# JettHuang/jet-pbrt

Hardware: AMD Instinct MI355X
Metric: Msamples/sec (whole node) + per-pixel L2 vs CPU ref, cornell_box 1024spp (higher is better)
Workload: dtype f32

## Files before the change

include/jetpbrt_amd.h:

```cpp
#ifndef JETPBRT_AMD_H
#define JETPBRT_AMD_H
#include <stdint.h>

#ifdef __cplusplus
extern "C" {
#endif

#define JP_ABI_VERSION 7

typedef enum JpStatus {
    JP_OK = 0,
    JP_ERR_INVALID_ARGUMENT = -1,
    JP_ERR_NO_DEVICE = -2,
    JP_ERR_DEVICE = -3,
    JP_ERR_NO_SCENE = -4,
    JP_ERR_UNSUPPORTED = -5
} JpStatus;

enum { JP_SHAPE_TRIANGLE = 0, JP_SHAPE_RECTANGLE = 1, JP_SHAPE_SPHERE = 2, JP_SHAPE_DISK = 3 };
enum { JP_MAT_MATTE = 0, JP_MAT_MIRROR = 1, JP_MAT_GLASS = 2, JP_MAT_PLASTIC = 3, JP_MAT_METAL = 4 };
enum { JP_LIGHT_ENVIRONMENT = 0, JP_LIGHT_AREA = 1, JP_LIGHT_POINT = 2, JP_LIGHT_DIRECTION = 3 };
enum { JP_SAMPLER_STOCK_MT19937 = 0, JP_SAMPLER_COUNTER = 1,
       JP_SAMPLER_DEBUG = 2 };
enum { JP_INTEGRATOR_PATH = 0, JP_INTEGRATOR_WHITTED = 1, JP_INTEGRATOR_DEBUG_NORMAL = 2 };
// ... 296 lines not shown
} JpTexSamplingInfo;
int  jp_set_texture_sampling(JpContext* ctx, const JpTextureSampling* sampling);
int  jp_check_texture_sampling(const JpTextureSampling* sampling, int32_t* n_active_textures, int32_t* n_active_maps);
int  jp_get_texture_sampling_info(JpContext* ctx, JpTexSamplingInfo* out);
int  jp_texture_lookup(const JpTexSampler* s_or_null, int32_t w, int32_t h, const uint8_t* rgb8, int32_t n, const float* uv, uint8_t* rgb8_out);
int  jp_perturb_normals_sampled(const JpTexSampler* s_or_null, int32_t n, const float* nb, const float* ng, const float* dpdu, const float* dpdv, const float* uv,
                                int32_t width, int32_t height, const uint8_t* rgb8, float strength, float* ns_out, int32_t* perturbed_out);

enum { JP_MIP_OFF = 0, JP_MIP_TRILINEAR = 1 };
typedef struct JpTextureMipmaps { int32_t struct_bytes, n_textures; const int32_t* mode; float footprint_scale, bounce_spread; } JpTextureMipmaps;
typedef struct JpTextureMipmapInfo {
    int32_t struct_bytes, n_on;
    int32_t n_levels;
    int32_t mip_last_render;
    int64_t pyramid_bytes_device;
    int64_t cone_bytes_device;
    double  build_ms;
    double  texel_ms;
    float   footprint_scale, bounce_spread, gamma0;
} JpTextureMipmapInfo;
int  jp_set_texture_mipmaps(JpContext* ctx, const JpTextureMipmaps* mipmaps);
int  jp_check_texture_mipmaps(const JpTextureMipmaps* mipmaps, int32_t* n_on);
int  jp_get_texture_mipmap_info(JpContext* ctx, JpTextureMipmapInfo* out);
int  jp_read_mip_chain(JpContext* ctx, int32_t texture, uint8_t* rgb8_out, int64_t capacity);
int  jp_build_mip_chain(int32_t w, int32_t h, const uint8_t* rgb8, uint8_t* rgb8_out, int32_t* level_w, int32_t* level_h, int32_t* n_levels);
int  jp_mip_cone_step(float gamma0, float bounce_spread, int32_t n, const int32_t* flags, const float* t, float* state_inout );
int  jp_mip_footprint(int32_t n, const float* width, const float* area, int32_t w, int32_t h, float scale_u, float scale_v, float footprint_scale, float* rho_out);
int  jp_texture_lookup_mip(const JpTexSampler* s_or_null, int32_t w, int32_t h, const uint8_t* rgb8, int32_t n, const float* uv, const float* rho, uint8_t* rgb8_out);
int  jp_mip_probe(JpContext* ctx, int32_t n, const float* origin, const float* dir, const float* tmin, const float* tmax, const int32_t* flags, float* state_inout,
                  int32_t* prim, float* rho, uint8_t* rgb8);

typedef struct JpLens { int32_t struct_bytes; float radius, focus_distance; int32_t blades; float rotation_deg; } JpLens;
int  jp_set_lens(JpContext* ctx, const JpLens* lens);
typedef struct JpLensInfo { int32_t struct_bytes; float radius, focus_distance; int32_t blades; float rotation_deg; int32_t lens_last_render; } JpLensInfo;
int  jp_get_lens_info(JpContext* ctx, JpLensInfo* out);
int  jp_check_lens(const JpLens* lens);
int  jp_lens_plan(const JpCamera* camera, const JpLens* lens, void* plan_out, int64_t capacity, int64_t* bytes);
int  jp_lens_rays(const JpCamera* camera, const JpLens* lens, int32_t n, const float* fxfy, const float* u, float* origin, float* dir);
int  jp_camera_rays(JpContext* ctx, const JpRenderParams* params, int32_t n, const int32_t* x, const int32_t* y, const int32_t* s, float* origin, float* dir, int32_t* dim_next);
int  jp_focus_distance(JpContext* ctx, float fx, float fy, float* focus_out);

typedef struct JpFilm { int32_t struct_bytes; int32_t hdr; float sample_clamp; } JpFilm;
int  jp_set_film(JpContext* ctx, const JpFilm* film);
int  jp_check_film(const JpFilm* film);
typedef struct JpFilmInfo { int32_t struct_bytes, hdr; float sample_clamp; int32_t hdr_last_render; } JpFilmInfo;
int  jp_get_film_info(JpContext* ctx, JpFilmInfo* out);
int  jp_film_samples(const JpFilm* film, int32_t n, const float* in_rgb, float* out_rgb);

#define JP_FILM_BINS 256
int  jp_film_histogram(JpContext* ctx, int32_t width, int32_t height, const float* film_rgb, uint32_t* hist);
int  jp_film_histogram_device(JpContext* ctx, int32_t width, int32_t height, const void* film_dev, void* hist_dev, int sync);

enum { JP_CURVE_CLAMP = 0, JP_CURVE_REINHARD = 1, JP_CURVE_ACES = 2, JP_CURVE_HABLE = 3 };
enum { JP_EXPOSURE_MANUAL = 0, JP_EXPOSURE_AUTO = 1 };
typedef struct JpToneMap { int32_t struct_bytes, curve, exposure_mode; float ev, key, white, pct_low, pct_high; } JpToneMap;
int  jp_set_tonemap(JpContext* ctx, const JpToneMap* tonemap);
int  jp_check_tonemap(const JpToneMap* tonemap);
int  jp_exposure_from_histogram(const JpToneMap* tonemap, const uint32_t* hist, float* scale_out);
int  jp_tonemap(JpContext* ctx, const JpToneMap* tonemap, int32_t width, int32_t height, const float* film_rgb, uint8_t* rgb8_out, float* rgb_out, float* scale_out);
int  jp_tonemap_device(JpContext* ctx, const JpToneMap* tonemap, int32_t width, int32_t height, const void* film_dev, void* rgb8_dev, void* rgb_dev, float* scale_out, int sync);
int  jp_tonemap_host(const JpToneMap* tonemap, float scale, int64_t n_values, const float* in, uint8_t* rgb8_out, float* rgb_out);
typedef struct JpToneMapInfo { int32_t struct_bytes, curve, exposure_mode; float scale_last; int32_t mapped_last_render; double histogram_ms, tonemap_ms; } JpToneMapInfo;
int  jp_get_tonemap_info(JpContext* ctx, JpToneMapInfo* out);

#define JP_UPLOAD_TABLES 11
typedef struct JpUploadTable { int64_t bytes; uint64_t fnv1a; } JpUploadTable;
typedef struct JpUploadInfo {
    int32_t struct_bytes;
    int32_t trav_mode;
    int32_t stack_depth, stack_depth_q4;
    int64_t lds_bytes, lds_bytes_shadow, shade_lds_bytes;
    int32_t scene_in_lds, tables_in_lds, shade_prims_in_lds, stage_nee, n_planes;
    int32_t persist, vote, shade_sort, use_q4, q4_shadow, cert;
    int32_t class_mask, shape_mask, light_mask, light_shape_mask;
    int32_t has_null_material, stack_lds_words;
    int32_t n_nodes, n_prims, n_flat, n_wide, n_q4;
    int32_t bvh_nodes, bvh_height;
    int32_t wide_height, q4_height, cert_eye_leaves, n_env;
    float   cert_pad, cert_pad_eye, env_sum[3];
    JpUploadTable table[JP_UPLOAD_TABLES];
} JpUploadInfo;
int  jp_describe_upload(const JpOptions* options_or_null, int32_t light_mode, const JpScene* scene, JpUploadInfo* out);

enum { JP_TABLE_NODES = 0, JP_TABLE_PRIMS = 1, JP_TABLE_META = 2, JP_TABLE_WIDE = 7, JP_TABLE_Q4 = 8, JP_TABLE_FLAT = 10 };
typedef struct JpTreeInfo {
    int32_t struct_bytes;
    int32_t n_prims, n_nodes, bvh_height;
    int32_t n_wide, wide_height;
    int32_t n_q4, q4_height;
    int32_t n_flat;
} JpTreeInfo;
int  jp_copy_upload_table(const JpOptions* options_or_null, int32_t light_mode, const JpScene* scene, int32_t which, void* out, int64_t capacity_bytes, int64_t* bytes);
int  jp_read_scene_table(JpContext* ctx, int32_t which, void* out, int64_t capacity_bytes, int64_t* bytes);
int  jp_get_tree_info(JpContext* ctx, JpTreeInfo* out);

#ifdef __cplusplus
}
#endif
#endif
```

jet-pbrt_amd/__init__.py:

```python
import ctypes as C
import os

PKG_DIR = os.path.dirname(os.path.abspath(__file__))
REPO_DIR = os.path.dirname(PKG_DIR)
HIP_LIB_PATH = os.environ.get("JETPBRT_AMD_LIB") or os.path.join(PKG_DIR, "csrc", "libjetpbrt_amd.so")
HOST_LIB_PATH = os.path.join(PKG_DIR, "host", "libjetpbrt_host.so")
CLI_PATH = os.path.join(PKG_DIR, "host", "jetpbrt")

JP_MAT_PARAM_STRIDE = 16
JP_SAMPLER_STOCK_MT19937, JP_SAMPLER_COUNTER, JP_SAMPLER_DEBUG = 0, 1, 2
JP_OK = 0

_fp = C.POINTER(C.c_float)
_ip = C.POINTER(C.c_int32)


class JpCamera(C.Structure):
    _fields_ = [("pos", C.c_float * 3), ("front", C.c_float * 3), ("right", C.c_float * 3), ("up", C.c_float * 3),
                ("res_x", C.c_float), ("res_y", C.c_float)]


class JpScene(C.Structure):
    _fields_ = [
        ("camera", JpCamera),
# ... 504 lines not shown
    if h is not None and h.size != JP_FILM_BINS + 1:
        raise JetPbrtError("exposure_from_histogram: the histogram has JP_FILM_BINS + 1 counts")
    s = C.c_float(0)
    L = hip_lib()
    _hip_status(L, L.jp_exposure_from_histogram(C.byref(t), None if h is None else h.ctypes.data_as(C.c_void_p), C.byref(s)))
    return s.value


def tonemap_host(t, scale, values, want_bytes=True, want_floats=True):
    import numpy as np
    a = np.ascontiguousarray(values, np.float32)
    b = np.zeros(a.shape, np.uint8) if want_bytes else None
    f = np.zeros(a.shape, np.float32) if want_floats else None
    q = lambda x: None if x is None else x.ctypes.data_as(C.c_void_p)
    L = hip_lib()
    _hip_status(L, L.jp_tonemap_host(C.byref(t), C.c_float(scale), a.size, q(a), q(b), q(f)))
    return b, f


def env_map(rgb, up_axis=JP_ENV_UP_Z, importance=0):
    import numpy as np
    a = np.ascontiguousarray(rgb, np.float32)
    if a.ndim != 3 or a.shape[2] != 3:
        raise JetPbrtError("an environment map is an (H, W, 3) array")
    m = JpEnvMap(C.sizeof(JpEnvMap), a.shape[1], a.shape[0], ENV_UP_AXES[up_axis], importance, a.ctypes.data_as(_fp))
    m._keep = a
    return m


def build_environment_table(rgb, tint=(1.0, 1.0, 1.0), up_axis=JP_ENV_UP_Z, importance=0):
    import numpy as np
    m = rgb if isinstance(rgb, JpEnvMap) else env_map(rgb, up_axis, importance)
    n = max(0, m.width) * max(0, m.height) if 0 < m.width <= 4096 and 0 < m.height <= 4096 else 0
    out = dict(weight=np.zeros(n, np.float64), q=np.zeros(n, np.float32), alias=np.zeros(n, np.int32), texel=np.zeros((n, 4), np.float32),
               row_cos=np.zeros((m.height if n else 0, 2), np.float32))
    t = np.ascontiguousarray(tint, np.float32)
    tot, mean = C.c_double(0.0), C.c_double(0.0)
    p = lambda a: a.ctypes.data_as(C.c_void_p)
    L = hip_lib()
    st = L.jp_build_environment_table(C.byref(m), p(t), p(out["weight"]), p(out["q"]), p(out["alias"]), p(out["texel"]), p(out["row_cos"]), C.byref(tot), C.byref(mean))
    if st != JP_OK:
        raise JetPbrtError("jetpbrt_amd status %d: %s" % (st, L.jp_last_error().decode()))
    out["total"], out["mean_sum"] = tot.value, mean.value
    return out


UPLOAD_TABLES = ("nodes", "prims", "meta", "mats", "mat_type", "lights", "shade_tab", "wide", "q4", "refbox", "flat")


class JpUploadTable(C.Structure):
    _fields_ = [("bytes", C.c_int64), ("fnv1a", C.c_uint64)]


class JpUploadInfo(C.Structure):
    _fields_ = [("struct_bytes", C.c_int32), ("trav_mode", C.c_int32), ("stack_depth", C.c_int32), ("stack_depth_q4", C.c_int32),
                ("lds_bytes", C.c_int64), ("lds_bytes_shadow", C.c_int64), ("shade_lds_bytes", C.c_int64),
                ("scene_in_lds", C.c_int32), ("tables_in_lds", C.c_int32), ("shade_prims_in_lds", C.c_int32), ("stage_nee", C.c_int32), ("n_planes", C.c_int32),
                ("persist", C.c_int32), ("vote", C.c_int32), ("shade_sort", C.c_int32), ("use_q4", C.c_int32), ("q4_shadow", C.c_int32), ("cert", C.c_int32),
                ("class_mask", C.c_int32), ("shape_mask", C.c_int32), ("light_mask", C.c_int32), ("light_shape_mask", C.c_int32),
                ("has_null_material", C.c_int32), ("stack_lds_words", C.c_int32),
                ("n_nodes", C.c_int32), ("n_prims", C.c_int32), ("n_flat", C.c_int32), ("n_wide", C.c_int32), ("n_q4", C.c_int32),
                ("bvh_nodes", C.c_int32), ("bvh_height", C.c_int32), ("wide_height", C.c_int32), ("q4_height", C.c_int32), ("cert_eye_leaves", C.c_int32), ("n_env", C.c_int32),
                ("cert_pad", C.c_float), ("cert_pad_eye", C.c_float), ("env_sum", C.c_float * 3),
                ("table", JpUploadTable * len(UPLOAD_TABLES))]


def describe_upload(scene, options=None, light_mode=JP_LIGHTS_ALL):
    L = hip_lib()
    info = JpUploadInfo()
    info.struct_bytes = C.sizeof(JpUploadInfo)
    if options is not None:
        options.struct_bytes = C.sizeof(JpOptions)
    st = L.jp_describe_upload(None if options is None else C.byref(options), LIGHT_SAMPLING_MODES[light_mode], scene if isinstance(scene, C._Pointer) else C.byref(scene), C.byref(info))
    if st != JP_OK:
        raise JetPbrtError("jetpbrt_amd status %d: %s" % (st, L.jp_last_error().decode()))
    return info


class JpTreeInfo(C.Structure):
    _fields_ = [("struct_bytes", C.c_int32), ("n_prims", C.c_int32), ("n_nodes", C.c_int32), ("bvh_height", C.c_int32), ("n_wide", C.c_int32), ("wide_height", C.c_int32),
                ("n_q4", C.c_int32), ("q4_height", C.c_int32), ("n_flat", C.c_int32)]


def _table_index(which):
    return UPLOAD_TABLES.index(which) if isinstance(which, str) else int(which)


def _read_table(call):
    import numpy as np
    n = C.c_int64(0)
    st = call(None, 0, C.byref(n))
    if st == JP_OK:
        out = np.zeros(n.value, np.uint8)
        if n.value:
            st = call(out.ctypes.data_as(C.c_void_p), n.value, C.byref(n))
    if st != JP_OK:
        raise JetPbrtError("jetpbrt_amd status %d: %s" % (st, hip_lib().jp_last_error().decode()))
    return out


def copy_upload_table(scene, which, options=None, light_mode=JP_LIGHTS_ALL):
    L = hip_lib()
    if options is not None:
        options.struct_bytes = C.sizeof(JpOptions)
    o = None if options is None else C.byref(options)
    sp = scene if isinstance(scene, C._Pointer) else C.byref(scene)
    return _read_table(lambda out, cap, n: L.jp_copy_upload_table(o, LIGHT_SAMPLING_MODES[light_mode], sp, _table_index(which), out, cap, n))


def build_light_table(weights):
    import numpy as np
    w = np.ascontiguousarray(weights, np.float64).reshape(-1)
    n = w.shape[0]
    q = np.zeros(n, np.float32); alias = np.zeros(n, np.int32); pmf = np.zeros(n, np.float32)
    p = lambda a: a.ctypes.data_as(C.c_void_p)
    L = hip_lib()
    st = L.jp_build_light_table(n, p(w), p(q), p(alias), p(pmf))
    if st != JP_OK:
        raise JetPbrtError("jetpbrt_amd status %d: %s" % (st, L.jp_last_error().decode()))
    return q, alias, pmf


def denoise_params(width, height, iterations=0, sigma_color=0.0, sigma_normal=0.0, sigma_depth=0.0, demodulate=0):
    return JpDenoiseParams(C.sizeof(JpDenoiseParams), width, height, iterations, sigma_color, sigma_normal, sigma_depth, demodulate)


def textures(tex_type, tex_color, mat_texture, n_triangles=0, tri_uv=None, images=()):
    import numpy as np
    n = len(tex_type)
    tt = np.ascontiguousarray(tex_type, np.int32); tc = np.ascontiguousarray(np.asarray(tex_color, np.float32).reshape(n, 6))
    w = np.zeros(n, np.int32); h = np.zeros(n, np.int32); off = np.zeros(n, np.int64)
    chunks, at = [], 0
    for k, img in dict(images).items():
        img = np.ascontiguousarray(img, np.uint8)
        h[k], w[k], off[k] = img.shape[0], img.shape[1], at
        chunks.append(img.reshape(-1)); at += img.size
    tx = np.ascontiguousarray(np.concatenate(chunks) if chunks else np.zeros(1, np.uint8))
    mt = np.ascontiguousarray(mat_texture, np.int32)
    t = JpTextures()
    t.struct_bytes = C.sizeof(JpTextures); t.n_textures = n
    t.tex_type = tt.ctypes.data_as(_ip); t.tex_color = tc.ctypes.data_as(_fp); t.tex_width = w.ctypes.data_as(_ip); t.tex_height = h.ctypes.data_as(_ip)
    t.tex_offset = off.ctypes.data_as(C.POINTER(C.c_int64)); t.n_texel_bytes = at; t.texels = tx.ctypes.data_as(C.POINTER(C.c_uint8))
    t.n_materials = len(mt); t.mat_texture = mt.ctypes.data_as(_ip); t.n_triangles = n_triangles
    uv = None
    if tri_uv is not None:
        uv = np.ascontiguousarray(tri_uv, np.float32); t.tri_uv = uv.ctypes.data_as(_fp)
    t._keep = (tt, tc, w, h, off, tx, mt, uv)
    return t


JP_BSDF_LAMBERT, JP_BSDF_MIRROR, JP_BSDF_FRESNEL_SPECULAR, JP_BSDF_MICROFACET_REFLECTION, JP_BSDF_MICROFACET_TRANSMISSION, JP_BSDF_PHONG = range(6)
JP_DIST_TROWBRIDGE_REITZ, JP_DIST_BECKMANN = 0, 1
JP_FRESNEL_CONDUCTOR, JP_FRESNEL_DIELECTRIC, JP_FRESNEL_NOOP = 0, 1, 2


def bsdf_desc(kind, color=(1, 1, 1), color2=(1, 1, 1), eta_a=1.0, eta_b=1.5, distribution=0, alpha=(0.2, 0.2), sample_visible=True, fresnel=0,
              fr_eta_i=(1, 1, 1), fr_eta_t=(1.5, 1.5, 1.5), fr_k=(0, 0, 0), exponent=10.0):
    d = JpBsdfDesc()
    d.kind = kind; d.color[:] = color; d.color2[:] = color2; d.eta_a = eta_a; d.eta_b = eta_b; d.distribution = distribution
    d.alpha_x, d.alpha_y = alpha; d.sample_visible = 1 if sample_visible else 0; d.fresnel = fresnel
    d.fr_eta_i[:] = fr_eta_i; d.fr_eta_t[:] = fr_eta_t; d.fr_k[:] = fr_k; d.exponent = exponent
    return d


def render_params(width, height, spp, max_depth=5, seed=1234, sampler_mode=JP_SAMPLER_COUNTER,
                  band_rows=20, shard_index=0, shard_count=1, integrator=JP_INTEGRATOR_PATH):
    return JpRenderParams(width, height, spp, max_depth, sampler_mode, seed, band_rows, shard_index, shard_count, integrator)
# ... 630 lines not shown
```

jet-pbrt_amd/csrc/jp_kernels.hip:

```cpp
#include "jp_common.h"
#include "jp_tex.h"
#include "jp_normals.h"
#include "jp_normal_map.h"
#include "jp_env.h"
#include "jp_mis.h"
#include "jp_lens.h"
#include "jp_xbsdf.h"
#include "jp_film.h"

#include <cstdio>
#include <cstring>
#include <string>
#include <vector>
#include <algorithm>
#include <cmath>
#include <mutex>
#include <thread>
#include <tuple>
#include <functional>
#include <type_traits>
#include "jp_devmem.h"
#include "jp_lbvh.h"
#include "jp_ploc.h"

// ... 131 lines not shown
{
	WalkStack stack;
	__device__ __forceinline__ SceneAccess(const SceneView&, int depth) { stack.lds = (int*)s_dyn + threadIdx.x; stack.spill = nullptr; stack.cap = depth - 1; stack.stride = 0; }
	template <bool kAnyHit> __device__ __forceinline__ int trace(const SceneView& sc, V3 o, V3 d, float tmin, float& tmax) const
	{ return walk_ray<6, kAnyHit>(sc, o, d, tmin, tmax, stack); }
};

template <> struct SceneAccess<5>
{
	const float4 *nodes, *prims; int* stack;
	__device__ __forceinline__ SceneAccess(const SceneView& sc, int) : nodes(sc.nodes), prims(sc.prims), stack((int*)s_dyn + threadIdx.x) {}
	template <bool kAnyHit> __device__ __forceinline__ int trace(const SceneView&, V3 o, V3 d, float tmin, float& tmax) const
	{ return traverse_ref<kAnyHit>(nodes, prims, o, d, tmin, tmax, stack); }
};

template <int kMode, typename F = FeatAll>
__global__ void __launch_bounds__(JP_BLOCK) k_extend(SceneView sc, Queues q, int cur, int depth, DevCounters* cnt)
{
	SceneAccess<kMode, F> acc(sc, depth);
	const unsigned int b = blockIdx.x, n = q.blk_q[cur][b], rbase = b * q.R;
	if (b == 0 && threadIdx.x == 0) { cnt->closest += cnt->n_queue[cur]; cnt->n_queue[cur ^ 1] = 0; cnt->n_shadow = 0; }
	unsigned int h = 0;
	float4 ro = make_float4(0, 0, 0, 0), rd = make_float4(0, 0, 1, 0);
	if (threadIdx.x < n) { ro = q.ray_o[cur][rbase + threadIdx.x]; rd = q.ray_d[cur][rbase + threadIdx.x]; }
	for (unsigned int j = threadIdx.x; j < n; j += JP_BLOCK)
	{
		const unsigned int i = rbase + j;
		const float4 co = ro, cd = rd;
		if (j + JP_BLOCK < n) { ro = q.ray_o[cur][i + JP_BLOCK]; rd = q.ray_d[cur][i + JP_BLOCK]; }
		float tmax = JP_INF;
		int hit;
		if constexpr (kMode == 2) hit = acc.trace_unbounded(sc, xyz(co), xyz(cd), 0.001f, tmax);
		else hit = acc.template trace<false>(sc, xyz(co), xyz(cd), 0.001f, tmax);
		q.hit[i] = make_float2(tmax, __int_as_float(hit));
		h += hit >= 0 ? 1u : 0u;
	}
	for (int off = 32; off > 0; off >>= 1) h += __shfl_down(h, off);
	if ((threadIdx.x & 63) == 0 && h) atomicAdd(&cnt->closest_hit, (unsigned long long)h);
}

struct PoolLds
{
	float4* rays; u64* slots; unsigned short* ring;
	__device__ __forceinline__ PoolLds(int n_prims)
	{
		char* base = (char*)(s_dyn + 5 * n_prims) + (threadIdx.x >> 6) * JP_POOL_WAVE_BYTES;
		rays = (float4*)base; slots = (u64*)(base + 64 * 32); ring = (unsigned short*)(base + 64 * 32 + 64 * 8);
	}
};

__global__ void __launch_bounds__(JP_BLOCK, 8) k_extend_pool(SceneView sc, Queues q, int cur, int depth, DevCounters* cnt)
{
	SceneAccess<2, FeatFlat> acc(sc, depth);
	const PoolLds pool(sc.n_prims);
	const unsigned int b = blockIdx.x, n = q.blk_q[cur][b], rbase = b * q.R;
	if (b == 0 && threadIdx.x == 0) { cnt->closest += cnt->n_queue[cur]; cnt->n_queue[cur ^ 1] = 0; cnt->n_shadow = 0; }
	unsigned int h = 0;
	float4 ro = make_float4(0, 0, 0, 0), rd = make_float4(0, 0, 1, 0);
	if (threadIdx.x < n) { ro = q.ray_o[cur][rbase + threadIdx.x]; rd = q.ray_d[cur][rbase + threadIdx.x]; }
	for (unsigned int j0 = threadIdx.x & ~63u; j0 < n; j0 += JP_BLOCK)
	{
		const unsigned int j = j0 + (threadIdx.x & 63u), i = rbase + j;
		const float4 co = ro, cd = rd;
		if (j + JP_BLOCK < n) { ro = q.ray_o[cur][i + JP_BLOCK]; rd = q.ray_d[cur][i + JP_BLOCK]; }
		float tmax = JP_INF;
		const unsigned int m = flat_boxes_lean<true>(sc.flat, sc.n_flat, xyz(co), xyz(cd), 0.001f, tmax);
		const int hit = flat_prims_pool<true, 5>(j < n ? m : 0u, acc.prims, xyz(co), xyz(cd), 0.001f, tmax, pool.rays, pool.slots, pool.ring);
		if (j < n) { q.hit[i] = make_float2(tmax, __int_as_float(hit)); h += hit >= 0 ? 1u : 0u; }
	}
	for (int off = 32; off > 0; off >>= 1) h += __shfl_down(h, off);
	if ((threadIdx.x & 63) == 0 && h) atomicAdd(&cnt->closest_hit, (unsigned long long)h);
}

#ifndef JP_SHADE_TILE
#define JP_SHADE_TILE 8192
#endif
template <bool kSmooth> struct SmoothVars { };
template <> struct SmoothVars<true> { float4 next, rec; V3 Ns; bool on, guard; };
template <bool kSmooth> __device__ __forceinline__ V3 shade_n(const SmoothVars<kSmooth>& sm, V3 N) { if constexpr (kSmooth) return sm.Ns; else return N; }
template <bool kSmooth> __device__ __forceinline__ bool shade_refuses(const SmoothVars<kSmooth>& sm, V3 w, V3 wo, V3 Ng)
{
	if constexpr (kSmooth) return sm.guard && dot(w, Ng) * dot(wo, Ng) <= 0.f; else return false;
}
template <bool kTab, bool kPrims, bool kStage, bool kSort, bool kTex, bool kPick, bool kEnv, bool kMis, typename F = FeatAll, bool kOne = false, bool kSmooth = false>
__device__ __forceinline__ void shade_body(SceneView sc, Queues q, RenderConst rc, int cur, DevCounters* cnt, const TexView& tv, const PickView& pv, const EnvView& ev, const MisView& mv, const NormView& nv = NormView())
{
	static_assert(kPick || !kMis, "k_shade: the light strategy's pdf needs the light table");
	static_assert(kTab || !kPrims, "k_shade: primitive records in LDS only together with the tables");
	static_assert(kPick || !kEnv, "k_shade: the map light is an entry of the light table");
	static_assert(!kSmooth || !kPrims, "k_shade: a shading normal has no entry in the frame table");
	constexpr int kWaves = JP_BLOCK / 64, kMaxSeg = (JP_SHADE_TILE / JP_BLOCK) * kWaves;
	static_assert(JP_SHADE_TILE % JP_BLOCK == 0 && JP_SHADE_TILE <= 65536, "k_shade: tile positions are 16-bit");
	__shared__ unsigned short s_idx[kSort ? JP_SHADE_TILE : 1];
	static_assert(!kOne || (kSort && kPrims && !F::delta && !F::other_lights && !kTex && !kPick && !kMis), "k_shade: the one-sweep partition is the lean sorted instance's");
	__shared__ unsigned char s_key[kSort && !kOne ? JP_SHADE_TILE : 1];
	__shared__ unsigned int s_cnt[kSort && !kOne ? JP_SHADE_CLASSES * kMaxSeg : 1];
	__shared__ unsigned int s_two;
	__shared__ unsigned int s_wsum[kWaves];
	__shared__ unsigned int s_ctr[3];
	const unsigned int lane = threadIdx.x & 63u;
	const int n_tab_l = kPick ? 0 : 2 * sc.n_lights;
	const int n_tab = n_tab_l + 4 * sc.n_mats + (sc.n_mats + 3) / 4, n_tab_all = n_tab + (kPrims ? 8 * sc.n_prims : 0);
	float4* s_lights = s_dyn;
	float4* s_mats = s_lights + n_tab_l;
	int* s_mtype = (int*)(s_mats + 4 * sc.n_mats);
	float4* s_prims = s_dyn + n_tab;
	int4* s_meta = (int4*)(s_prims + 4 * sc.n_prims);
	const float4* s_frames = s_prims + 5 * sc.n_prims;
	float4* s_stage = s_dyn + n_tab_all + threadIdx.x;
	const unsigned int b = blockIdx.x, n = q.blk_q[cur][b];
	const int nxt = cur ^ 1;
#ifdef JP_SHADE_TIMING
	unsigned long long t_acc[10] = { 0, 0, 0, 0, 0, 0, 0, 0, 0, 0 }, t_last = __builtin_amdgcn_s_memtime();
#endif
	if (kTab)
	{
		for (int i = threadIdx.x; i < n_tab_all; i += 2 * JP_BLOCK)
		{
			const bool two = i + JP_BLOCK < n_tab_all;
			const float4 a = sc.shade_tab[i], c2 = two ? sc.shade_tab[i + JP_BLOCK] : a;
			s_dyn[i] = a; if (two) s_dyn[i + JP_BLOCK] = c2;
		}
	}
	if (n == 0) { if (threadIdx.x == 0) { q.blk_q[nxt][b] = 0; q.blk_sh[b] = 0; } return; }
	if (threadIdx.x == 0) { s_ctr[0] = 0; s_ctr[1] = 0; s_ctr[2] = 0; if (kOne) s_two = 0; }
	__syncthreads();
	const float4* lights = (kTab && !kPick) ? (const float4*)s_lights : sc.lights;
	const float4* mats = kTab ? (const float4*)s_mats : sc.mats;
	const int* mat_type = kTab ? (const int*)s_mtype : sc.mat_type;
	const float4* prims = kPrims ? (const float4*)s_prims : sc.prims;
	const int4* meta_t = kPrims ? (const int4*)s_meta : sc.meta;
	const unsigned int rbase = b * q.R;
	const unsigned int t0 = 0, count = n;
	JP_TS(0);
	if (kOne)
	{
		const unsigned int tid = threadIdx.x, npass = (count + JP_BLOCK - 1) / JP_BLOCK;
		const unsigned long long ltm = (1ull << lane) - 1ull;
		#pragma unroll 1
		for (unsigned int r0 = 0; r0 < npass; r0 += 8)
		{
			int pi[8];
			#pragma unroll
			for (int u = 0; u < 8; u++)
			{
				const unsigned int j = (r0 + u) * JP_BLOCK + tid;
				pi[u] = j < count ? __float_as_int(q.hit[rbase + t0 + j].y) : -2;
			}
			int mt[8]; unsigned long long ma[8], mb[8];
			unsigned int na = 0, nb = 0;
			#pragma unroll
			for (int u = 0; u < 8; u++)
			{
				mt[u] = -1;
				if (pi[u] >= 0) { const int m = meta_t[pi[u]].y; if (m >= 0) mt[u] = mat_type[m]; }
				ma[u] = __ballot(mt[u] == JP_MAT_MATTE); mb[u] = __ballot(mt[u] == JP_MAT_METAL);
				na += (unsigned int)__popcll(ma[u]); nb += (unsigned int)__popcll(mb[u]);
			}
			if (na | nb)
			{
				const unsigned int base = wave_take(&s_two, na | (nb << 16));
				unsigned int a = base & 0xffffu, m = base >> 16;
				#pragma unroll
				for (int u = 0; u < 8; u++)
				{
					const unsigned short j = (unsigned short)((r0 + u) * JP_BLOCK + tid);
					if (mt[u] == JP_MAT_MATTE) s_idx[a + (unsigned int)__popcll(ma[u] & ltm)] = j;
					if (mt[u] == JP_MAT_METAL) s_idx[count - 1u - (m + (unsigned int)__popcll(mb[u] & ltm))] = j;
					a += (unsigned int)__popcll(ma[u]); m += (unsigned int)__popcll(mb[u]);
				}
			}
		}
		__syncthreads();
	}
	else if (kSort)
	{
		constexpr unsigned int seg = kMaxSeg, nctr = JP_SHADE_CLASSES * kMaxSeg;
		const unsigned int tid = threadIdx.x;
		const unsigned int plane = tid & 63u, wave = tid >> 6, npass = (count + JP_BLOCK - 1) / JP_BLOCK;
		const unsigned long long ltm = (1ull << plane) - 1ull;
		#pragma unroll 1
		for (unsigned int r0 = 0; r0 < npass; r0 += 8)
		{
			int pi[8];
			#pragma unroll
			for (int u = 0; u < 8; u++)
			{
				const unsigned int j = (r0 + u) * JP_BLOCK + tid;
				pi[u] = j < count ? __float_as_int(q.hit[rbase + t0 + j].y) : -2;
			}
			#pragma unroll
			for (int u = 0; u < 8; u++)
			{
				const unsigned int r = r0 + u;
				if (r >= npass) break;
				unsigned int key = JP_SHADE_CLASSES;
				if (pi[u] != -2)
				{
					int m = -1; if (pi[u] >= 0) m = meta_t[pi[u]].y;
					key = m >= 0 ? 1u + (unsigned int)mat_type[m] : 0u;
				}
				s_key[r * JP_BLOCK + tid] = (unsigned char)key;
				unsigned int mine = 0;
				#pragma unroll
				for (int c = 0; c < JP_SHADE_CLASSES; c++)
				{
					unsigned int nc = 0;
					if ((rc.class_mask >> c) & 1) nc = (unsigned int)__popcll(__ballot(key == (unsigned int)c));
					if (plane == (unsigned int)c) mine = nc;
				}
				if (plane < JP_SHADE_CLASSES) s_cnt[plane * seg + r * kWaves + wave] = mine;
			}
		}
		__syncthreads();
		{
			static_assert(JP_SHADE_CLASSES * kMaxSeg <= 3 * JP_BLOCK, "k_shade: three counters per thread");
			unsigned int v[3], t = 0;
			#pragma unroll
			for (int i = 0; i < 3; i++)
			{
				const unsigned int at = 3 * tid + i;
				v[i] = (at < nctr && (at % seg) / kWaves < npass) ? s_cnt[at] : 0u; t += v[i];
			}
			unsigned int incl = t;
			#pragma unroll
			for (int off = 1; off < 64; off <<= 1) { const unsigned int o = __shfl_up(incl, off); if (plane >= (unsigned int)off) incl += o; }
			if (plane == 63) s_wsum[wave] = incl;
			__syncthreads();
			unsigned int base = incl - t;
			#pragma unroll
			for (int w = 0; w < kWaves; w++) if ((unsigned int)w < wave) base += s_wsum[w];
			#pragma unroll
			for (int i = 0; i < 3; i++) { const unsigned int at = 3 * tid + i; if (at < nctr) s_cnt[at] = base; base += v[i]; }
		}
		__syncthreads();
		#pragma unroll 1
		for (unsigned int r = 0; r < npass; r++)
		{
			const unsigned int key = s_key[r * JP_BLOCK + tid];
			unsigned int pre = 0;
			#pragma unroll
			for (int c = 0; c < JP_SHADE_CLASSES; c++)
			{
				if (!((rc.class_mask >> c) & 1)) continue;
				const unsigned long long m = __ballot(key == (unsigned int)c);
				if (key == (unsigned int)c) pre = (unsigned int)__popcll(m & ltm);
			}
			if (key < JP_SHADE_CLASSES) s_idx[s_cnt[key * seg + r * kWaves + wave] + pre] = (unsigned short)(r * JP_BLOCK + tid);
		}
		__syncthreads();
	}
	SmoothVars<kSmooth> sm;
	if constexpr (kSmooth) sm.next = make_float4(0, 0, 0, 0);
	float4 ro_n = make_float4(0, 0, 0, 0), rd_n = ro_n, rb_n = ro_n; float2 h_n = make_float2(0, 0); unsigned int s_n = 0; float2 m_n = make_float2(0, 0);
	JP_TS(1);
	const unsigned int n_front = kOne ? (s_two & 0xffffu) : 0u, n_back = kOne ? (s_two >> 16) : 0u, fence = ((n_front + 63u) >> 6) << 6;
#define JP_CHUNK_HAS(v)  (kOne ? ((v) < fence ? (v) < n_front : (v) - fence < n_back) : (v) < count)
#define JP_CHUNK_SPOT(v) (kOne ? ((v) < fence ? (v) : count - 1u - ((v) - fence)) : (v))
	const unsigned int nch = kOne ? (fence >> 6) + ((n_back + 63u) >> 6) : (count + 63u) >> 6;
	unsigned int tk = wave_take(&s_ctr[0], 1u);
	unsigned int c0 = (nch - 1u - tk) << 6;
	if (tk < nch && JP_CHUNK_HAS(c0 + lane)) { const unsigned int pos = JP_CHUNK_SPOT(c0 + lane), i0 = rbase + t0 + (kSort ? (unsigned int)s_idx[pos] : pos); ro_n = q.ray_o[cur][i0]; rd_n = q.ray_d[cur][i0]; rb_n = q.beta[cur][i0]; h_n = q.hit[i0]; if (kTex) s_n = tv.side[i0]; if (kMis) m_n = mv.side[cur][i0]; if constexpr (kSmooth) sm.next = nv.side[i0]; }
	while (tk < nch)
	{
		const bool valid = JP_CHUNK_HAS(c0 + lane);
#ifdef JP_SHADE_TIMING
		JP_TS(2);
		asm volatile("s_waitcnt vmcnt(0)" ::: "memory");
		JP_TS(3);
#endif
#ifdef JP_SHADE_NO_PREFETCH
		if (valid) { const unsigned int pos = JP_CHUNK_SPOT(c0 + lane), i0 = rbase + t0 + (kSort ? (unsigned int)s_idx[pos] : pos); ro_n = q.ray_o[cur][i0]; rd_n = q.ray_d[cur][i0]; rb_n = q.beta[cur][i0]; h_n = q.hit[i0]; if (kTex) s_n = tv.side[i0]; if (kMis) m_n = mv.side[cur][i0]; if constexpr (kSmooth) sm.next = nv.side[i0]; }
		const float4 ro = ro_n, rd = rd_n, rb = rb_n; const float2 h = h_n; const unsigned int sw = s_n; const float2 ms = m_n;
		if constexpr (kSmooth) sm.rec = sm.next;
		tk = wave_take(&s_ctr[0], 1u); c0 = (nch - 1u - tk) << 6;
#else
		const float4 ro = ro_n, rd = rd_n, rb = rb_n; const float2 h = h_n; const unsigned int sw = s_n; const float2 ms = m_n;
		if constexpr (kSmooth) sm.rec = sm.next;
		tk = wave_take(&s_ctr[0], 1u); c0 = (nch - 1u - tk) << 6;
		if (tk < nch && JP_CHUNK_HAS(c0 + lane))
		{
			const unsigned int pos = JP_CHUNK_SPOT(c0 + lane);
			const unsigned int i1 = rbase + t0 + (kSort ? (unsigned int)s_idx[pos] : pos);
			ro_n = q.ray_o[cur][i1]; rd_n = q.ray_d[cur][i1]; rb_n = q.beta[cur][i1]; h_n = q.hit[i1]; if (kTex) s_n = tv.side[i1]; if (kMis) m_n = mv.side[cur][i1]; if constexpr (kSmooth) sm.next = nv.side[i1];
// ... 996 lines not shown
```

jet-pbrt_amd/csrc/jp_normal_map.h:

```cpp
#ifndef JP_NORMAL_MAP_DEVICE_PART
#define JP_NORMAL_MAP_DEVICE_PART
#include "jp_common.h"
#include "jp_tex.h"
#include "jp_normals.h"
#include "../../include/jp_normal_map.h"
#include "jp_tex_sampling.h"

struct NMapView
{
	const int4* desc;
	const unsigned int* texels;
	const float2* mat;
	const float2* prim_uv;
};

namespace jp
{
__device__ __forceinline__ V3 hit_normal(const float4* prims, int h, V3 p, V3 rd)
{
	const float4 g3 = prims[4 * h + 3]; const int type = __float_as_int(g3.w);
	if (type == JP_SHAPE_TRIANGLE) return xyz(g3);
	if (type == JP_SHAPE_RECTANGLE) return dot(xyz(g3), rd) <= 0 ? xyz(g3) : -xyz(g3);
	if (type == JP_SHAPE_DISK) return xyz(prims[4 * h + 1]);
	return normalize(p - xyz(prims[4 * h]));
// ... 117 lines not shown
		ng[3 * i] = N.x; ng[3 * i + 1] = N.y; ng[3 * i + 2] = N.z;
		ns[3 * i] = Ns.x; ns[3 * i + 1] = Ns.y; ns[3 * i + 2] = Ns.z;
	}
}

namespace
{
typedef void (*ShadingNormalMappedKernel)(SceneView, NormView, NMapView, SampView, int, int, const float*, const float*, const float*, const float*, int*, float*, float*);
ShadingNormalMappedKernel shading_normal_mapped_kernel(const TraceLaunch& t) { return by_trace_mode(t.mode, [](auto m) -> ShadingNormalMappedKernel { return k_shading_normal_mapped<decltype(m)::value>; }); }

int check_normal_maps(const JpNormalMaps* m, long long& pool, int& n_mapped)
{
	pool = 0; n_mapped = 0;
	if (m->struct_bytes < (int32_t)sizeof(JpNormalMaps)) return fail(JP_ERR_INVALID_ARGUMENT, "jp_set_normal_maps: set JpNormalMaps.struct_bytes to sizeof(JpNormalMaps)");
	if (m->n_maps < 0 || m->n_maps > (1 << 28)) return fail(JP_ERR_INVALID_ARGUMENT, "jp_set_normal_maps: n_maps out of range");
	if (m->n_materials < 0 || m->n_triangles < 0) return fail(JP_ERR_INVALID_ARGUMENT, "jp_set_normal_maps: negative n_materials or n_triangles");
	if (m->n_maps > 0 && (!m->map_width || !m->map_height || !m->map_offset || !m->texels)) return fail(JP_ERR_INVALID_ARGUMENT, "jp_set_normal_maps: null map_width / map_height / map_offset / texels");
	if (m->n_materials > 0 && !m->mat_map) return fail(JP_ERR_INVALID_ARGUMENT, "jp_set_normal_maps: null mat_map");
	for (int i = 0; i < m->n_maps; i++)
	{
		const long long w = m->map_width[i], h = m->map_height[i], off = m->map_offset[i];
		if (w < 1 || w > 16384 || h < 1 || h > 16384) return fail(JP_ERR_INVALID_ARGUMENT, "jp_set_normal_maps: map " + std::to_string(i) + ": size out of range (1 .. 16384 per side)");
		if (off < 0 || m->n_texel_bytes < 0 || off > m->n_texel_bytes - 3 * w * h) return fail(JP_ERR_INVALID_ARGUMENT, "jp_set_normal_maps: map " + std::to_string(i) + ": texels beyond n_texel_bytes");
		pool += w * h;
	}
	if (pool > 0x7fffffffll) return fail(JP_ERR_INVALID_ARGUMENT, "jp_set_normal_maps: more than 2^31 texels in all");
	for (int k = 0; k < m->n_materials; k++)
	{
		if (m->mat_map[k] < -1 || m->mat_map[k] >= m->n_maps) return fail(JP_ERR_INVALID_ARGUMENT, "jp_set_normal_maps: material " + std::to_string(k) + ": mat_map out of range");
		if (m->mat_strength && !std::isfinite(m->mat_strength[k])) return fail(JP_ERR_INVALID_ARGUMENT, "jp_set_normal_maps: material " + std::to_string(k) + ": strength not finite");
		if (m->mat_map[k] >= 0) n_mapped++;
	}
	if (m->tri_uv) for (size_t k = 0; k < 6 * (size_t)m->n_triangles; k++) if (!std::isfinite(m->tri_uv[k])) return fail(JP_ERR_INVALID_ARGUMENT, "jp_set_normal_maps: triangle " + std::to_string(k / 6) + ": uv not finite");
	return JP_OK;
}

float bits_as_float(int i) { float f; std::memcpy(&f, &i, sizeof(f)); return f; }
void pack_rgb8(const uint8_t* src, size_t n, unsigned int* dst)
{
	for (size_t k = 0; k < n; k++) dst[k] = (unsigned int)src[3 * k] | ((unsigned int)src[3 * k + 1] << 8) | ((unsigned int)src[3 * k + 2] << 16) | 0xff000000u;
}
}

static int upload_normal_maps(JpContext* c, SceneTables& T, ScenePlan& plan, const JpScene* s)
{
	const NormalMapsHost& m = c->nmaps;
	if (m.n_materials != s->n_materials) return fail(JP_ERR_INVALID_ARGUMENT, "jp_upload_scene: the normal maps' n_materials differs from the scene's (jp_set_normal_maps)");
	if (m.n_triangles != s->n_triangles) return fail(JP_ERR_INVALID_ARGUMENT, "jp_upload_scene: the normal maps' n_triangles differs from the scene's (jp_set_normal_maps)");
	plan.nm_maps = (int)m.width.size(); plan.nm_mapped = m.n_mapped; plan.nm_texel_bytes = plan.nm_table_bytes = 0;
	std::vector<float2> mat((size_t)std::max(1, s->n_materials), make_float2(bits_as_float(-1), 0.f));
	int effective = 0;
	for (int k = 0; k < s->n_materials; k++)
	{
		const int i = m.mat_map[k]; const float st = m.strength.empty() ? 1.f : m.strength[k];
		if (i < 0 || m.neutral[i] || st == 0.f) continue;
		mat[k] = make_float2(bits_as_float(i), st); effective++;
	}
	if (effective == 0) return JP_OK;
	std::vector<int4> desc(m.width.size());
	for (size_t i = 0; i < desc.size(); i++) desc[i] = make_int4(m.width[i], m.height[i], (int)m.first[i], 0);
	HIP_TRY(upload(T.nm_desc, desc.data(), desc.size() * sizeof(int4)));
	HIP_TRY(upload(T.nm_texels, m.texels.data(), m.texels.size() * sizeof(unsigned int)));
	HIP_TRY(upload(T.nm_mat, mat.data(), mat.size() * sizeof(float2)));
	NMapView mp = {}; mp.desc = T.nm_desc.get<int4>(); mp.texels = T.nm_texels.get<unsigned int>(); mp.mat = T.nm_mat.get<float2>();
	plan.nm_table_bytes = (long long)(desc.size() * sizeof(int4) + mat.size() * sizeof(float2));
	if (!m.tri_uv.empty() && s->n_primitives > 0)
	{
		std::vector<float2> puv(3 * (size_t)s->n_primitives, make_float2(0.f, 0.f));
		for (int p = 0; p < s->n_primitives; p++)
			if (s->prim_shape_type[p] == JP_SHAPE_TRIANGLE)
			{
				const float* u = m.tri_uv.data() + 6 * (size_t)s->prim_shape_index[p];
				for (int k = 0; k < 3; k++) puv[3 * (size_t)p + k] = make_float2(u[2 * k], u[2 * k + 1]);
			}
		HIP_TRY(upload(T.nm_prim_uv, puv.data(), puv.size() * sizeof(float2)));
		mp.prim_uv = T.nm_prim_uv.get<float2>();
		plan.nm_table_bytes += (long long)(puv.size() * sizeof(float2));
	}
	plan.nm_texel_bytes = (long long)(m.texels.size() * sizeof(unsigned int));
	plan.mp = mp; plan.mapped = true;
	if (!plan.smooth)
	{
		plan.nv = NormView(); plan.smooth = true;
		plan.tables_in_lds = false; plan.shade_prims_in_lds = false; plan.stage_nee = false; plan.shade_lds_bytes = 0;
	}
	return JP_OK;
}

extern "C" {

int jp_check_normal_maps(const JpNormalMaps* m, int32_t* n_mapped_materials)
{
	if (!m) return fail(JP_ERR_INVALID_ARGUMENT, "jp_check_normal_maps: null argument");
	long long pool; int nm;
	const int st = check_normal_maps(m, pool, nm);
	if (st == JP_OK && n_mapped_materials) *n_mapped_materials = nm;
	return st;
}

int jp_set_normal_maps(JpContext* c, const JpNormalMaps* m)
{
	if (!c) return fail(JP_ERR_INVALID_ARGUMENT, "jp_set_normal_maps: null context");
	if (!m) { c->nmaps = NormalMapsHost(); return JP_OK; }
	long long pool; int nm;
	if (const int st = check_normal_maps(m, pool, nm); st != JP_OK) return st;
	NormalMapsHost h; h.set = true; h.n_materials = m->n_materials; h.n_triangles = m->n_triangles; h.n_mapped = nm;
	h.texels.resize((size_t)pool);
	size_t at = 0;
	for (int i = 0; i < m->n_maps; i++)
	{
		const size_t n = (size_t)m->map_width[i] * (size_t)m->map_height[i];
		const uint8_t* src = m->texels + m->map_offset[i];
		h.width.push_back(m->map_width[i]); h.height.push_back(m->map_height[i]); h.first.push_back((long long)at);
		pack_rgb8(src, n, h.texels.data() + at);
		bool neutral = true;
		for (size_t k = 0; k < n && neutral; k++) neutral = src[3 * k] == 128 && src[3 * k + 1] == 128;
		h.neutral.push_back(neutral ? 1 : 0);
		at += n;
	}
	if (m->n_materials > 0) h.mat_map.assign(m->mat_map, m->mat_map + m->n_materials);
	if (m->mat_strength && m->n_materials > 0) h.strength.assign(m->mat_strength, m->mat_strength + m->n_materials);
	if (m->tri_uv && m->n_triangles > 0) h.tri_uv.assign(m->tri_uv, m->tri_uv + 6 * (size_t)m->n_triangles);
	c->nmaps = std::move(h);
	return JP_OK;
}

int jp_get_normal_map_info(JpContext* c, JpNormalMapInfo* out)
{
	if (!c || !out) return fail(JP_ERR_INVALID_ARGUMENT, "jp_get_normal_map_info: null argument");
	if (out->struct_bytes < (int32_t)sizeof(int32_t)) return fail(JP_ERR_INVALID_ARGUMENT, "jp_get_normal_map_info: set JpNormalMapInfo.struct_bytes to sizeof(JpNormalMapInfo)");
	JpNormalMapInfo i; std::memset(&i, 0, sizeof(i));
	if (c->plan.have_scene) { i.n_maps = c->plan.nm_maps; i.n_mapped_materials = c->plan.nm_mapped; i.texel_bytes_device = c->plan.nm_texel_bytes; i.table_bytes_device = c->plan.nm_table_bytes; }
	i.mapped_last_render = c->last_nmapped;
	if (c->profiling && c->last_nmapped)
	{
		if (const int st = finish_counters(c); st != JP_OK) return st;
		i.normal_map_ms = c->normal_map_ms; for (int k = 1; k < c->last_lanes; k++) i.normal_map_ms += c->lanes[k - 1]->normal_map_ms;
	}
	const size_t n = std::min((size_t)out->struct_bytes, sizeof(i));
	i.struct_bytes = (int32_t)n;
	std::memcpy(out, &i, n);
	return JP_OK;
}

int jp_perturb_normals(int32_t n, const float* nb, const float* ng, const float* dpdu, const float* dpdv, const float* uv,
                       int32_t width, int32_t height, const uint8_t* rgb8, float strength, float* ns_out, int32_t* perturbed_out)
{
	if (n < 0 || (n > 0 && (!nb || !ng || !dpdu || !dpdv || !uv || !ns_out || !perturbed_out)) || !rgb8) return fail(JP_ERR_INVALID_ARGUMENT, "jp_perturb_normals: null argument");
	if (width < 1 || width > 16384 || height < 1 || height > 16384) return fail(JP_ERR_INVALID_ARGUMENT, "jp_perturb_normals: size out of range (1 .. 16384 per side)");
	std::vector<unsigned int> texels((size_t)width * (size_t)height);
	pack_rgb8(rgb8, texels.size(), texels.data());
	for (int32_t i = 0; i < n; i++)
	{
		const size_t k = 3 * (size_t)i;
		float ns[3] = { nb[k], nb[k + 1], nb[k + 2] };
		perturbed_out[i] = jp_perturb_normal(nb + k, ng + k, dpdu + k, dpdv + k, uv[2 * (size_t)i], uv[2 * (size_t)i + 1], texels.data(), width, height, strength, ns);
		ns_out[k] = ns[0]; ns_out[k + 1] = ns[1]; ns_out[k + 2] = ns[2];
	}
	return JP_OK;
}

int jp_triangle_tangents(int32_t n, const float* p0, const float* p1, const float* p2, const float* uv6, float* dpdu, float* dpdv, int32_t* ok_out)
{
	if (n < 0 || (n > 0 && (!p0 || !p1 || !p2 || !uv6 || !dpdu || !dpdv || !ok_out))) return fail(JP_ERR_INVALID_ARGUMENT, "jp_triangle_tangents: null argument");
	for (int32_t i = 0; i < n; i++)
	{
		const size_t k = 3 * (size_t)i;
// ... 10 lines not shown
```

jet-pbrt_amd/csrc/jp_normals.h:

```cpp
#ifndef JP_NORMALS_DEVICE_PART
#define JP_NORMALS_DEVICE_PART
#include "jp_common.h"
#include "../../include/jp_normals.h"

struct NormView
{
	const float4* prim_vn;
	float4* side;
};

namespace jp
{
__device__ __forceinline__ bool shading_normal(const float4* prims, const NormView& nv, int h, int prim, V3 p, V3& Ns)
{
	const float4 g3 = prims[4 * h + 3];
	if (__float_as_int(g3.w) != JP_SHAPE_TRIANGLE) return false;
	const float4 v0 = nv.prim_vn[3 * prim], v1 = nv.prim_vn[3 * prim + 1], v2 = nv.prim_vn[3 * prim + 2];
	if (v0.w == 0.f) return false;
	const float4 g0 = prims[4 * h], g1 = prims[4 * h + 1], g2 = prims[4 * h + 2];
	const float a0[3] = { g0.x, g0.y, g0.z }, a1[3] = { g1.x, g1.y, g1.z }, a2[3] = { g2.x, g2.y, g2.z }, ng[3] = { g3.x, g3.y, g3.z }, ap[3] = { p.x, p.y, p.z };
	const float vn9[9] = { v0.x, v0.y, v0.z, v1.x, v1.y, v1.z, v2.x, v2.y, v2.z };
	float ns[3];
	jp_shading_normal_at(a0, a1, a2, ng, vn9, ap, ns);
	Ns = mk(ns[0], ns[1], ns[2]);
// ... 35 lines not shown
{ const EnvView ev = {}; const MisView mv = {}; JP_SMOOTH_BODY(kSort, true, true, false, false); }
template <bool kSort> __global__ void __launch_bounds__(JP_BLOCK, 3) k_shade_smooth_env(SceneView sc, Queues q, RenderConst rc, int cur, DevCounters* cnt, PickView pv, EnvView ev, NormView nv)
{ const TexView tv = {}; const MisView mv = {}; JP_SMOOTH_BODY(kSort, false, true, true, false); }
template <bool kSort> __global__ void __launch_bounds__(JP_BLOCK, 3) k_shade_smooth_env_tex(SceneView sc, Queues q, RenderConst rc, int cur, DevCounters* cnt, TexView tv, PickView pv, EnvView ev, NormView nv)
{ const MisView mv = {}; JP_SMOOTH_BODY(kSort, true, true, true, false); }
template <bool kSort> __global__ void __launch_bounds__(JP_BLOCK, 3) k_shade_smooth_mis(SceneView sc, Queues q, RenderConst rc, int cur, DevCounters* cnt, PickView pv, MisView mv, NormView nv)
{ const TexView tv = {}; const EnvView ev = {}; JP_SMOOTH_BODY(kSort, false, true, false, true); }
template <bool kSort> __global__ void __launch_bounds__(JP_BLOCK, 3) k_shade_smooth_mis_tex(SceneView sc, Queues q, RenderConst rc, int cur, DevCounters* cnt, TexView tv, PickView pv, MisView mv, NormView nv)
{ const EnvView ev = {}; JP_SMOOTH_BODY(kSort, true, true, false, true); }
template <bool kSort> __global__ void __launch_bounds__(JP_BLOCK, 3) k_shade_smooth_mis_env(SceneView sc, Queues q, RenderConst rc, int cur, DevCounters* cnt, PickView pv, EnvView ev, MisView mv, NormView nv)
{ const TexView tv = {}; JP_SMOOTH_BODY(kSort, false, true, true, true); }
template <bool kSort> __global__ void __launch_bounds__(JP_BLOCK, 3) k_shade_smooth_mis_env_tex(SceneView sc, Queues q, RenderConst rc, int cur, DevCounters* cnt, TexView tv, PickView pv, EnvView ev, MisView mv, NormView nv)
{ JP_SMOOTH_BODY(kSort, true, true, true, true); }
#undef JP_SMOOTH_BODY

template <int kMode>
__global__ void __launch_bounds__(JP_BLOCK) k_shading_normal(SceneView sc, NormView nv, int smooth, int depth, int n, const float* o, const float* d, const float* tmin, const float* tmax_in,
                                                                int* prim, float* ng, float* ns)
{
	SceneAccess<kMode> acc(sc, depth);
	for (int i = blockIdx.x * JP_BLOCK + threadIdx.x; i < n; i += gridDim.x * JP_BLOCK)
	{
		const V3 ro = mk(o[3 * i], o[3 * i + 1], o[3 * i + 2]), rd = mk(d[3 * i], d[3 * i + 1], d[3 * i + 2]);
		float tmax = tmax_in[i];
		const int h = acc.template trace<false>(sc, ro, rd, tmin[i], tmax);
		V3 N = mk(0, 0, 0), Ns = N; int pr = -1;
		if (h >= 0)
		{
			const float4 g3 = sc.prims[4 * h + 3]; const int type = __float_as_int(g3.w);
			const V3 p = ro + tmax * rd;
			pr = sc.meta[h].x;
			if (type == JP_SHAPE_TRIANGLE) N = xyz(g3);
			else if (type == JP_SHAPE_RECTANGLE) N = dot(xyz(g3), rd) <= 0 ? xyz(g3) : -xyz(g3);
			else if (type == JP_SHAPE_DISK) N = xyz(sc.prims[4 * h + 1]);
			else N = normalize(p - xyz(sc.prims[4 * h]));
			Ns = N;
			if (smooth) shading_normal(sc.prims, nv, h, pr, p, Ns);
		}
		prim[i] = pr;
		ng[3 * i] = N.x; ng[3 * i + 1] = N.y; ng[3 * i + 2] = N.z;
		ns[3 * i] = Ns.x; ns[3 * i + 1] = Ns.y; ns[3 * i + 2] = Ns.z;
	}
}

namespace
{
typedef void (*ShadingNormalKernel)(SceneView, NormView, int, int, int, const float*, const float*, const float*, const float*, int*, float*, float*);
ShadingNormalKernel shading_normal_kernel(const TraceLaunch& t) { return by_trace_mode(t.mode, [](auto m) -> ShadingNormalKernel { return k_shading_normal<decltype(m)::value>; }); }

int check_vertex_normals(int n, const float* vn, int& n_smooth)
{
	n_smooth = 0;
	for (int i = 0; i < n; i++)
	{
		const int k = jp_vertex_normals_class(vn + 9 * (size_t)i);
		if (k < 0)
		{
			bool finite = true; for (int j = 0; j < 9; j++) if (!std::isfinite(vn[9 * (size_t)i + j])) finite = false;
			return fail(JP_ERR_INVALID_ARGUMENT, "jp_set_vertex_normals: triangle " + std::to_string(i) + (finite ? ": a normal's squared length is outside [0.81, 1.21] (nine zeros mark a flat triangle)" : ": a value is not finite"));
		}
		n_smooth += k;
	}
	return JP_OK;
}
}

static int upload_vertex_normals(JpContext* c, SceneTables& T, ScenePlan& plan, const JpScene* s)
{
	const VertexNormalsHost& v = c->vnormals;
	if (v.n_triangles != s->n_triangles) return fail(JP_ERR_INVALID_ARGUMENT, "jp_upload_scene: the vertex normals' n_triangles differs from the scene's (jp_set_vertex_normals)");
	c->vn_triangles = v.n_triangles; c->vn_smooth = v.n_smooth; c->vn_table_bytes = 0;
	if (v.n_smooth == 0) return JP_OK;
	std::vector<float4> rec(3 * (size_t)std::max(1, s->n_primitives), make_float4(0.f, 0.f, 0.f, 0.f));
	for (int p = 0; p < s->n_primitives; p++)
	{
		if (s->prim_shape_type[p] != JP_SHAPE_TRIANGLE) continue;
		const float* n9 = v.vn.data() + 9 * (size_t)s->prim_shape_index[p];
		if (jp_vertex_normals_class(n9) != 1) continue;
		for (int k = 0; k < 3; k++) rec[3 * (size_t)p + k] = make_float4(n9[3 * k], n9[3 * k + 1], n9[3 * k + 2], k == 0 ? 1.f : 0.f);
	}
	HIP_TRY(upload(T.prim_vn, rec.data(), rec.size() * sizeof(float4)));
	plan.nv = NormView(); plan.nv.prim_vn = T.prim_vn.get<float4>();
	plan.smooth = true;
	plan.tables_in_lds = false; plan.shade_prims_in_lds = false; plan.stage_nee = false; plan.shade_lds_bytes = 0;
	c->vn_table_bytes = (long long)(rec.size() * sizeof(float4));
	return JP_OK;
}

static int ensure_normal_side(JpContext* c, unsigned int cap, NormView& nv)
{
	if (const int e = reserve_idle(c, c->nside, (size_t)cap * sizeof(float4)); e != JP_OK) return e;
	nv.side = c->nside.get<float4>();
	return JP_OK;
}

extern "C" {

int jp_set_vertex_normals(JpContext* c, const JpVertexNormals* vn)
{
	if (!c) return fail(JP_ERR_INVALID_ARGUMENT, "jp_set_vertex_normals: null context");
	if (!vn) { c->vnormals = VertexNormalsHost(); return JP_OK; }
	if (vn->struct_bytes < (int32_t)sizeof(JpVertexNormals)) return fail(JP_ERR_INVALID_ARGUMENT, "jp_set_vertex_normals: set JpVertexNormals.struct_bytes to sizeof(JpVertexNormals)");
	if (vn->n_triangles < 0 || (vn->n_triangles > 0 && !vn->tri_vn)) return fail(JP_ERR_INVALID_ARGUMENT, "jp_set_vertex_normals: bad n_triangles or null tri_vn");
	int ns = 0;
	if (const int st = check_vertex_normals(vn->n_triangles, vn->tri_vn, ns); st != JP_OK) return st;
	VertexNormalsHost h; h.set = true; h.n_triangles = vn->n_triangles; h.n_smooth = ns;
	h.vn.assign(vn->tri_vn, vn->tri_vn + 9 * (size_t)vn->n_triangles);
	c->vnormals = std::move(h);
	return JP_OK;
}

int jp_get_normal_info(JpContext* c, JpNormalInfo* out)
{
	if (!c || !out) return fail(JP_ERR_INVALID_ARGUMENT, "jp_get_normal_info: null argument");
	if (out->struct_bytes < (int32_t)sizeof(int32_t)) return fail(JP_ERR_INVALID_ARGUMENT, "jp_get_normal_info: set JpNormalInfo.struct_bytes to sizeof(JpNormalInfo)");
	JpNormalInfo i; std::memset(&i, 0, sizeof(i));
	if (c->plan.have_scene) { i.n_triangles = c->vn_triangles; i.n_smooth_triangles = c->vn_smooth; i.table_bytes_device = c->vn_table_bytes; }
	i.smooth_last_render = c->last_smooth;
	if (c->profiling && c->last_smooth)
	{
		if (const int st = finish_counters(c); st != JP_OK) return st;
		i.normal_ms = c->normal_ms; for (int k = 1; k < c->last_lanes; k++) i.normal_ms += c->lanes[k - 1]->normal_ms;
	}
	const size_t n = std::min((size_t)out->struct_bytes, sizeof(i));
	i.struct_bytes = (int32_t)n;
	std::memcpy(out, &i, n);
	return JP_OK;
}

int jp_interpolate_normals(int32_t n, const float* p0, const float* p1, const float* p2, const float* ng, const float* vn9, const float* p, float* ns_out)
{
	if (n < 0 || (n > 0 && (!p0 || !p1 || !p2 || !ng || !vn9 || !p || !ns_out))) return fail(JP_ERR_INVALID_ARGUMENT, "jp_interpolate_normals: null argument");
	for (int32_t i = 0; i < n; i++) jp_shading_normal_at(p0 + 3 * (size_t)i, p1 + 3 * (size_t)i, p2 + 3 * (size_t)i, ng + 3 * (size_t)i, vn9 + 9 * (size_t)i, p + 3 * (size_t)i, ns_out + 3 * (size_t)i);
	return JP_OK;
}

int jp_check_vertex_normals(const JpVertexNormals* vn, int32_t* n_smooth)
{
	if (!vn) return fail(JP_ERR_INVALID_ARGUMENT, "jp_check_vertex_normals: null argument");
	if (vn->struct_bytes < (int32_t)sizeof(JpVertexNormals)) return fail(JP_ERR_INVALID_ARGUMENT, "jp_set_vertex_normals: set JpVertexNormals.struct_bytes to sizeof(JpVertexNormals)");
	if (vn->n_triangles < 0 || (vn->n_triangles > 0 && !vn->tri_vn)) return fail(JP_ERR_INVALID_ARGUMENT, "jp_set_vertex_normals: bad n_triangles or null tri_vn");
	int ns = 0;
	const int st = check_vertex_normals(vn->n_triangles, vn->tri_vn, ns);
	if (st == JP_OK && n_smooth) *n_smooth = ns;
	return st;
}

int jp_shading_normal(JpContext* c, int32_t n, const float* origin, const float* dir, const float* tmin, const float* tmax, int32_t* prim, float* ng, float* ns)
{
	if (!c || n < 0 || !origin || !dir || !tmin || !tmax || !prim || !ng || !ns) return fail(JP_ERR_INVALID_ARGUMENT, "jp_shading_normal: null argument");
	if (!c->plan.have_scene) return fail(JP_ERR_NO_SCENE, "jp_shading_normal: no scene uploaded");
	if (n == 0) return JP_OK;
	const TraceLaunch tk = trace_kernel(c->plan, c->opt.trace_walk, true);
	const ShadingNormalKernel k = shading_normal_kernel(tk);
	const ShadingNormalMappedKernel km = c->plan.mapped ? shading_normal_mapped_kernel(tk) : nullptr;
	if (!k || (c->plan.mapped && !km)) return fail(JP_ERR_UNSUPPORTED, "jp_shading_normal: no instance for this scene's walk");
	HIP_TRY(hipSetDevice(c->device));
	DevBuf b_in, b_g, b_s, b_prim; float *d_in, *d_g, *d_s; int* d_prim;
	HIP_TRY(reserve(b_in, d_in, (size_t)n * 32)); HIP_TRY(reserve(b_g, d_g, (size_t)n * 12)); HIP_TRY(reserve(b_s, d_s, (size_t)n * 12)); HIP_TRY(reserve(b_prim, d_prim, (size_t)n * 4));
	float *d_o = d_in, *d_d = d_in + 3 * (size_t)n, *d_t0 = d_in + 6 * (size_t)n, *d_t1 = d_in + 7 * (size_t)n;
	HIP_TRY(hipMemcpyAsync(d_o, origin, (size_t)n * 12, hipMemcpyHostToDevice, c->stream)); HIP_TRY(hipMemcpyAsync(d_d, dir, (size_t)n * 12, hipMemcpyHostToDevice, c->stream));
	HIP_TRY(hipMemcpyAsync(d_t0, tmin, (size_t)n * 4, hipMemcpyHostToDevice, c->stream)); HIP_TRY(hipMemcpyAsync(d_t1, tmax, (size_t)n * 4, hipMemcpyHostToDevice, c->stream));
	const int grid = std::min(c->n_cus * 8, (n + JP_BLOCK - 1) / JP_BLOCK);
	if (km) hipLaunchKernelGGL(km, dim3(grid), dim3(JP_BLOCK), tk.lds, c->stream, c->plan.sv, c->plan.nv, c->plan.mp, c->plan.sm, tk.depth, n, (const float*)d_o, (const float*)d_d, (const float*)d_t0, (const float*)d_t1, d_prim, d_g, d_s);
	else hipLaunchKernelGGL(k, dim3(grid), dim3(JP_BLOCK), tk.lds, c->stream, c->plan.sv, c->plan.nv, c->plan.smooth ? 1 : 0, tk.depth, n, (const float*)d_o, (const float*)d_d, (const float*)d_t0, (const float*)d_t1, d_prim, d_g, d_s);
	HIP_TRY(hipGetLastError());
	HIP_TRY(hipMemcpyAsync(prim, d_prim, (size_t)n * 4, hipMemcpyDeviceToHost, c->stream)); HIP_TRY(hipMemcpyAsync(ng, d_g, (size_t)n * 12, hipMemcpyDeviceToHost, c->stream));
// ... 8 lines not shown
```

jet-pbrt_amd/csrc/jp_render.h:

```cpp
#pragma once
namespace
{
enum { CLS_EXTEND = 0, CLS_SHADE = 1, CLS_SHADOW = 2, CLS_OTHER = 3, CLS_PATH = 4, CLS_NORMAL = 5, CLS_NMAP = 6, CLS_TEXEL = 7 };

int lens_plan_of(const JpContext* c, JpLensPlan& lp)
{
	std::memset(&lp, 0, sizeof(lp));
	if (!c->lens_on) return JP_OK;
	if (jp_lens_make_plan(&c->plan.sv.cam, &c->lens, &lp) != 0) return fail(JP_ERR_INVALID_ARGUMENT, "jp_set_lens: the uploaded camera's right / up vectors have no finite positive length");
	return JP_OK;
}

void free_queues(JpContext* c) { c->qb = QueueBufs(); c->cap = 0; c->planes_alloc = 0; c->blk_alloc = 0; }

int ensure_queues(JpContext* c, unsigned int cap, int planes, unsigned int nblocks)
{
	if (c->cap >= cap && c->planes_alloc >= planes && c->blk_alloc >= nblocks) return JP_OK;
	cap = std::max(cap, c->cap); planes = std::max(planes, c->planes_alloc); nblocks = std::max(nblocks, c->blk_alloc);
	free_queues(c);
	auto alloc = [](DevBuf& b, auto*& p, size_t bytes) { return reserve(b, p, bytes) == hipSuccess; };
	Queues& q = c->q; QueueBufs& qb = c->qb; bool ok = true;
	for (int b = 0; b < 2 && ok; b++) ok = alloc(qb.ray_o[b], q.ray_o[b], (size_t)cap * 16) && alloc(qb.ray_d[b], q.ray_d[b], (size_t)cap * 16) && alloc(qb.beta[b], q.beta[b], (size_t)cap * 16)
	                                       && alloc(qb.blk_q[b], q.blk_q[b], (size_t)nblocks * 4);
	ok = ok && alloc(qb.hit, q.hit, (size_t)cap * 8) && alloc(qb.lacc, q.lacc, (size_t)cap * 16) && alloc(qb.sh_o, q.sh_o, (size_t)cap * 16)
// ... 227 lines not shown
		if (c->opt.max_slots > 0) budget = std::min<size_t>(budget, (size_t)c->opt.max_slots * per);
		int sbatch = 1; unsigned int P = 0, G = 1, R = JP_BLOCK, cap = 0;
		for (int attempt = 0;; attempt++)
		{
			const unsigned int pcap = (unsigned int)std::min<size_t>(PMAX, std::max<size_t>((size_t)npix, budget / per));
			sbatch = (int)std::max<long long>(1, std::min<long long>(rp->spp, pcap / npix));
			{
				const int nb = (rp->spp + sbatch - 1) / sbatch;
				sbatch = (rp->spp + nb - 1) / nb;
			}
			if ((long long)sbatch * npix > (long long)PMAX) return fail(JP_ERR_UNSUPPORTED, "jp_render: shard too large for one batch");
			P = (unsigned int)((long long)sbatch * npix);
			const unsigned int nchunks = (P + JP_BLOCK - 1) / JP_BLOCK;
			G = std::max(1u, std::min(nchunks, (unsigned int)(c->n_cus * c->blocks_per_cu)));
			G = std::max(G, (nchunks + JP_SHADE_TILE / JP_BLOCK - 1) / (JP_SHADE_TILE / JP_BLOCK));
			R = ((nchunks + G - 1) / G) * JP_BLOCK;
			cap = G * R;
			const int st = ensure_queues(c, cap, p.n_planes, G);
			if (st == JP_OK) break;
			if (sbatch <= 1 || attempt >= 6) return st;
			budget = (size_t)sbatch / 2 * (size_t)npix * per;
		}
		c->q.cap = cap; c->q.R = R;
		const bool tex = p.textured && rp->integrator == JP_INTEGRATOR_PATH;
		if (tex) if (const int e = reserve_idle(c, c->side, (size_t)cap * sizeof(unsigned int)); e != JP_OK) return e;
		TexView tv = p.tv; tv.side = c->side.get<unsigned int>();
		MipView mv_cone = {};
		if (tex && p.mip_on > 0) { mv_cone = p.mv; if (const int e = ensure_cone(c, cap, mv_cone); e != JP_OK) return e; }
		const bool mis = c->estimator == JP_ESTIMATOR_MIS && rp->integrator == JP_INTEGRATOR_PATH;
		MisView mv = {};
		if (mis) if (const int e = ensure_mis_side(c, cap, mv); e != JP_OK) return e;
		NormView nv = p.nv;
		if (smooth) if (const int e = ensure_normal_side(c, cap, nv); e != JP_OK) return e;
		if (const int e = reserve_idle(c, c->spill, spill_need(p, p.persist ? deepest_walk(p) : 0, G) * sizeof(int)); e != JP_OK) return e;
		if (const int e = reserve_idle(c, c->pix_acc, (size_t)npix * 16); e != JP_OK) return e;
		int* const d_spill = c->spill.get<int>(); float4* const d_pix_acc = c->pix_acc.get<float4>();

		RenderConst rc; rc.width = rp->width; rc.height = rp->height; rc.spp = rp->spp; rc.max_depth = rp->max_depth; rc.seed = rp->seed;
		rc.band_rows = sh.band; rc.shard_index = sh.index; rc.shard_count = sh.count; rc.npix = (int)npix; rc.local_rows = sh.lane_rows; rc.n_planes = p.n_planes;
		rc.lane_index = lane_index; rc.lane_count = lane_count; rc.lane_rows = lane_group; rc.class_mask = p.class_mask; rc.sampler_debug = rp->sampler_mode == JP_SAMPLER_DEBUG ? 1 : 0;
		rc.slot_bits = slot_bits;
		rc.tiled = 0;
		rc.compact = (p.trav_mode != 2 && p.trav_mode != 1 && npix % JP_BLOCK == 0) ? 1 : 0;
		if (c->opt.compact_regions != 0) rc.compact = (c->opt.compact_regions > 0 && npix % JP_BLOCK == 0) ? 1 : 0;
		const int grid = (int)G;
		const bool generic = c->opt.reserved[0] == 1;
		const ExtendLaunch ek = extend_kernel(p, generic); const ShadowLaunch sk = shadow_kernel(p, R, generic); const OtherKernel ok = other_kernel(p);
		const ShadeLaunch shade = shade_launch(shade_choice(p, tex, mis, smooth, generic), ShadeViews(tv, p.pv, p.ev, mv, nv));
		JpLensPlan lp;
		if (const int e = lens_plan_of(c, lp); e != JP_OK) return e;
		for (int s0 = 0; s0 < rp->spp; s0 += sbatch)
		{
			rc.s0 = s0; rc.sbatch = std::min(sbatch, rp->spp - s0);
			{
				Stamper t(c, CLS_OTHER);
				if (c->lens_on) hipLaunchKernelGGL(k_raygen<true>, dim3(grid), dim3(JP_BLOCK), 0, c->stream, p.sv, c->q, rc, d_cnt, lp);
				else hipLaunchKernelGGL(k_raygen<false>, dim3(grid), dim3(JP_BLOCK), 0, c->stream, p.sv, c->q, rc, d_cnt, NoLens());
			}
			if (rp->integrator != JP_INTEGRATOR_PATH)
			{
				Stamper t(c, CLS_OTHER);
				const int ogrid = (int)std::min<unsigned int>((P + JP_BLOCK - 1) / JP_BLOCK, (unsigned int)(c->n_cus * 16));
				hipLaunchKernelGGL(ok, dim3(ogrid), dim3(JP_BLOCK), p.lds_bytes, c->stream, p.sv, c->q, rc, rp->integrator, p.stack_depth, d_cnt, c->lens_on ? 1 : 0, lp);
			}
			int cur = 0;
			int iters = rp->integrator != JP_INTEGRATOR_PATH ? 0 : rp->max_depth + 1;
			for (int it = 0;; it++)
			{
				if (it >= iters)
				{
					if (rp->integrator != JP_INTEGRATOR_PATH || !p.has_null_material || it > iters + 64) break;
					DevCounters h; HIP_TRY(hipMemcpyAsync(&h, d_cnt, sizeof(h), hipMemcpyDeviceToHost, c->stream)); HIP_TRY(hipStreamSynchronize(c->stream));
					if (h.n_queue[cur] == 0) break;
				}
				{
					Stamper t(c, CLS_EXTEND);
					if (ek.refill) hipLaunchKernelGGL(ek.refill, dim3(grid), dim3(JP_BLOCK), ek.lds, c->stream, p.sv, c->q, cur, ek.words, d_spill, d_cnt);
					else hipLaunchKernelGGL(ek.plain, dim3(grid), dim3(JP_BLOCK), ek.lds, c->stream, p.sv, c->q, cur, ek.words, d_cnt);
				}
				{
					Stamper t(c, CLS_SHADE);
					if (tex) launch_texel(c, p, grid, cur, tv, mv_cone);
					if (smooth) launch_normal(c, p, grid, cur, nv);
					shade(c->stream, grid, p.shade_lds_bytes, p.sv, c->q, rc, cur, d_cnt);
				}
				HIP_TRY(hipGetLastError());
				if (it < rp->max_depth || p.has_null_material)
				{
					Stamper t(c, CLS_SHADOW);
					if (sk.cert_fell_back) c->cert_fell_back = true;
					if (sk.refill) hipLaunchKernelGGL(sk.refill, dim3(grid), dim3(JP_BLOCK), sk.lds, c->stream, p.sv, c->q, rc, sk.words, d_spill, d_cnt);
					else hipLaunchKernelGGL(sk.plain, dim3(grid), dim3(JP_BLOCK), sk.lds, c->stream, p.sv, c->q, rc, sk.words, d_cnt);
					HIP_TRY(hipGetLastError());
				}
				cur ^= 1;
			}
			{ Stamper t(c, CLS_OTHER); launch_resolve(c, c->q, rc, npix, d_pix_acc, film_dev, s0 == 0 ? 1 : 0, s0 + rc.sbatch >= rp->spp ? 1 : 0); }
			samples += (unsigned long long)rc.sbatch * (unsigned long long)npix;
		}
		HIP_TRY(hipGetLastError());
	}
	HIP_TRY(hipEventRecord(c->ev1, c->stream));
	c->own_samples = samples;
	if (sync) HIP_TRY(hipStreamSynchronize(c->stream));
	return JP_OK;
}

__global__ void __launch_bounds__(JP_BLOCK) k_add_film(float* __restrict__ dst, const float* __restrict__ src, size_t n)
{
	for (size_t i = (size_t)blockIdx.x * JP_BLOCK + threadIdx.x; i < n; i += (size_t)gridDim.x * JP_BLOCK) dst[i] += src[i];
}

int make_lanes(JpContext* c, int extra)
{
	if (!c->ev_added && hipEventCreateWithFlags(&c->ev_added, hipEventDisableTiming) != hipSuccess) return fail(JP_ERR_DEVICE, "jp_render: event allocation failed");
	while ((int)c->lanes.size() < extra)
	{
		JpContext* l = new JpContext;
		l->device = c->device; l->is_lane = true; l->n_cus = c->n_cus; l->blocks_per_cu = c->blocks_per_cu; l->opt = c->opt; l->opt_env = c->opt_env;
		std::memset(&l->counters, 0, sizeof(l->counters)); std::memset(&l->q, 0, sizeof(l->q));
		if (hipStreamCreateWithFlags(&l->stream, hipStreamNonBlocking) != hipSuccess || hipEventCreate(&l->ev0) != hipSuccess || hipEventCreate(&l->ev1) != hipSuccess
		    || l->cnt.reserve(sizeof(DevCounters)) != hipSuccess)
		{ jp_destroy_context(l); return fail(JP_ERR_DEVICE, "jp_render: stream/event allocation for an extra lane failed"); }
		c->lanes.push_back(l);
	}
	return JP_OK;
}

void sync_lane_scene(JpContext* c, JpContext* l)
{
	l->plan = c->plan;
	if (!l->plan.textured && l->side) { hipStreamSynchronize(l->stream); l->side.reset(); }
	if (l->plan.mip_on == 0 && l->cone) { hipStreamSynchronize(l->stream); l->cone.reset(); }
	if (!l->plan.smooth && l->nside) { hipStreamSynchronize(l->stream); l->nside.reset(); }
	l->profiling = c->profiling; l->opt = c->opt;
	l->estimator = c->estimator;
	l->lens = c->lens; l->lens_on = c->lens_on;
	l->film_state = c->film_state; l->film_on = c->film_on;
}

bool fused_eligible(const JpContext* c, const JpRenderParams* rp)
{
	if (c->opt.fused <= 0) return false;
	if (c->is_lane || !c->plan.have_scene || rp->integrator != JP_INTEGRATOR_PATH) return false;
	if (!c->plan.tables_in_lds || c->plan.n_planes > 4) return false;
	if (c->plan.cert) return false;
	if (c->plan.textured) return false;
	if (c->plan.pick) return false;
	if (c->plan.smooth) return false;
	if (c->lens_on) return false;
	if (c->plan.trav_mode == 2) return c->plan.shade_prims_in_lds;
	return c->plan.trav_mode == 0 || c->plan.trav_mode == 3 || c->plan.trav_mode == 5;
}

typedef void (*PathKernel)(SceneView, Queues, RenderConst, PathConst, int*, DevCounters*);
PathKernel path_kernel(const ScenePlan& p)
{
	const bool so = p.shade_sort;
	switch (p.trav_mode)
	{
	case 2: return so ? k_path<2, 2, true, true, true> : k_path<2, 2, true, false, true>;
	case 3:
		if (p.use_q4) return p.q4_shadow ? (so ? k_path<4, 4, false, true, true> : k_path<4, 4, false, false, true>) : (so ? k_path<4, 3, false, true, true> : k_path<4, 3, false, false, true>);
		return so ? k_path<0, 3, false, true, true> : k_path<0, 3, false, false, true>;
	case 5: return so ? k_path<5, 5, false, true, false> : k_path<5, 5, false, false, false>;
	default:
		if (p.use_q4) return so ? k_path<4, 4, false, true, true> : k_path<4, 4, false, false, true>;
// ... 435 lines not shown
```

jet-pbrt_amd/csrc/jp_runtime.h:

```cpp
#pragma once

static thread_local std::string g_err;
static int fail(int code, const std::string& msg) { g_err = msg; return code; }
#define HIP_TRY(expr) do { hipError_t _e = (expr); if (_e != hipSuccess) return fail(JP_ERR_DEVICE, std::string(#expr) + ": " + hipGetErrorString(_e)); } while (0)

static inline bool opt_flag(int v, bool dflt) { return v == 0 ? dflt : v > 0; }

static void options_from_environment(JpOptions& o)
{
	struct Item { const char* name; int kind; void* field; int as; };
	const Item items[] = {
		{ "JETPBRT_LANES", 0, &o.lanes, 0 }, { "JETPBRT_LANE_ROWS", 0, &o.lane_rows, 0 }, { "JETPBRT_BLOCKS_PER_CU", 0, &o.blocks_per_cu, 0 }, { "JETPBRT_MAX_SLOTS", 3, &o.max_slots, 0 },
		{ "JETPBRT_COMPACT_REGIONS", 1, &o.compact_regions, 0 }, { "JETPBRT_FUSED", 1, &o.fused, 0 }, { "JETPBRT_REGION", 0, &o.fused_region, 0 }, { "JETPBRT_JOB_SPP", 0, &o.fused_job_spp, 0 },
		{ "JETPBRT_FUSED_WGS", 0, &o.fused_workgroups, 0 }, { "JETPBRT_TRAVERSAL", 6, &o.traversal, 0 }, { "JETPBRT_Q4", 1, &o.q4, 0 }, { "JETPBRT_Q4_SHADOW", 1, &o.q4_shadow, 0 },
		{ "JETPBRT_PERSIST", 2, &o.persist, 0 }, { "JETPBRT_VOTE", 1, &o.vote, 0 }, { "JETPBRT_STACK_LDS", 0, &o.stack_lds_words, 0 }, { "JETPBRT_SHADE_SORT", 1, &o.shade_sort, 0 },
		{ "JETPBRT_DEVICE_TREE", 4, &o.device_tree, 0 }, { "JETPBRT_DEVICE_WIDE", 1, &o.device_wide, 0 }, { "JETPBRT_BVH_MAXLEAF", 0, &o.bvh_max_leaf, 0 },
		{ "JETPBRT_PLOC_RADIUS", 0, &o.ploc_radius, 0 }, { "JETPBRT_PLOC_MAX_ROUNDS", 0, &o.ploc_max_rounds, 0 }, { "JETPBRT_CERTIFIED", 1, &o.certified, 0 },
		{ "JETPBRT_CERT_SLACK", 7, &o.cert_slack, 0 }, { "JETPBRT_CERT_SLACK_EYE", 7, &o.cert_slack_eye, 0 }, { "JETPBRT_CERT_EYE", 7, &o.cert_eye_tau, 0 },
		{ "JETPBRT_SINCOSF", 2, &o.libm_sincosf, 0 }, { "JETPBRT_LIBM", 2, &o.libm_xbsdf, 0 },
		{ "JETPBRT_TRACE_BINARY", 5, &o.trace_walk, 1 }, { "JETPBRT_TRACE_WIDE", 5, &o.trace_walk, 2 }, { "JETPBRT_TRACE_VERBATIM", 5, &o.trace_walk, 3 }, { "JETPBRT_BOX_PAD", 7, &o.box_pad, 0 },
	};
	for (const Item& it : items)
	{
		const char* e = getenv(it.name);
		if (!e || !*e) continue;
		switch (it.kind)
		{
			case 0: *(int32_t*)it.field = atoi(e); break;
			case 1: *(int32_t*)it.field = atoi(e) != 0 ? 1 : -1; break;
			case 2: { const int v = atoi(e); *(int32_t*)it.field = v != 0 ? v : -1; break; }
			case 3: *(int64_t*)it.field = atoll(e); break;
			case 4: *(int32_t*)it.field = std::string(e) == "lbvh" ? 2 : 1; break;
			case 5: *(int32_t*)it.field = it.as; break;
			case 6: { const int v = atoi(e); if (v >= 0 && v <= 3) *(int32_t*)it.field = 1 + v; break; }
			case 7: { const float v = (float)atof(e); *(float*)it.field = v != 0.f ? v : -1.f; break; }
		}
	}
}

struct ScenePlan
{
	bool have_scene = false;
	SceneView sv; TexView tv = {}; bool textured = false;
	PickView pv = {}; bool pick = false;
	NormView nv = {}; bool smooth = false;
	NMapView mp = {}; bool mapped = false;
	int nm_maps = 0, nm_mapped = 0; long long nm_texel_bytes = 0, nm_table_bytes = 0;
	SampView sm = {}; int ts_active_textures = 0, ts_active_maps = 0; long long ts_table_bytes = 0;
	MipView mv = {}; int mip_on = 0, mip_levels = 0; long long mip_bytes = 0;
	EnvView ev = {}; bool env = false; double env_mean_sum = 0.0;
	int trav_mode = 0, stack_depth = 1, stack_depth_q4 = 0; bool scene_in_lds = false, shade_prims_in_lds = false; size_t lds_bytes = 0, lds_bytes_shadow = 0;
	bool cert = false;
	bool use_q4 = false, q4_shadow = false;
	bool vote = false; int persist = 0;
	int n_planes = 1; bool has_null_material = false;
	bool tables_in_lds = false, stage_nee = false; size_t shade_lds_bytes = 0;
	int class_mask = 0x3f; bool shade_sort = false;
	int shape_mask = 0xf, light_mask = 0xf, light_shape_mask = 0xf;
	int stack_lds_words = 12;
};

struct SceneTables
{
	DevBuf nodes, prims, meta, mats, mat_type, lights, shade_tab, flat, wide, q4, refbox;
	DevBuf tex_desc, tex_col, texels, mat_tex, prim_uv;
	DevBuf pick_bins, pick_pmf, pick_env;
	DevBuf env_texel, env_bins, env_rows;
	DevBuf prim_vn;
	DevBuf nm_desc, nm_texels, nm_mat, nm_prim_uv;
	DevBuf ts_tex, ts_map;
	DevBuf mip_tex, mip_lev;
};
struct QueueBufs { DevBuf ray_o[2], ray_d[2], beta[2], blk_q[2], hit, lacc, sh_o, sh_d, sh_c, blk_sh; };

struct EnvMapHost { int W = 0, H = 0, up = 0, importance = 0; std::vector<float> rgb; };
struct VertexNormalsHost { bool set = false; int n_triangles = 0, n_smooth = 0; std::vector<float> vn; };

struct NormalMapsHost { bool set = false; int n_materials = 0, n_triangles = 0, n_mapped = 0; std::vector<int> width, height, mat_map; std::vector<long long> first; std::vector<char> neutral;
                        std::vector<unsigned int> texels; std::vector<float> strength, tri_uv; };

struct TexSamplingHost { bool has_tex = false, has_map = false; int n_textures = 0, n_maps = 0, n_active_textures = 0, n_active_maps = 0; std::vector<JpTexSampler> tex, map; };

struct MipmapsHost { bool set = false; int n_textures = 0, n_on = 0; float footprint_scale = 0.f, bounce_spread = 0.f; std::vector<int32_t> mode; };

struct JpContext
{
	int device = 0;
	JpOptions opt{}, opt_env{};
	hipStream_t stream = nullptr;
	int n_cus = 256;
	ScenePlan plan; SceneTables tab;
	bool cert_fell_back = false; int cert_eye_leaves = 0;
	int sincosf_mode = 0, libm_mode = 0;
	bool build_on_device = false; float build_ms = 0.f; int bvh_height = 0, bvh_nodes = 0;
	int wide_height = 0, q4_height = 0; size_t tab_bytes[JP_UPLOAD_TABLES] = {};
	Queues q = {}; QueueBufs qb; unsigned int cap = 0; int planes_alloc = 0; unsigned int blk_alloc = 0; int blocks_per_cu = 16;
	DevBuf pix_acc, spill, film;
	DevBuf bsdf_in, bsdf_out, bsdf_fl;
	DevBuf gamma, rgb8; PinnedBuf h_rgb8;
	PinnedBuf h_film;
	DevBuf cnt;
	hipEvent_t ev0 = nullptr, ev1 = nullptr;
	bool profiling = false;
	std::vector<hipEvent_t> evpool; size_t evused = 0;
	struct Stamp { int cls; size_t a, b; };
	std::vector<Stamp> stamps;
	JpCounters counters;
	std::vector<JpContext*> lanes; bool is_lane = false; unsigned long long own_samples = 0; bool bpc_from_env = false;
	hipEvent_t ev_added = nullptr; bool added_valid = false; int last_lanes = 1;
	Queues fq = {}; QueueBufs fqb; unsigned int fcap = 0; int fplanes = 0;
	DevBuf jobs;
	int last_fused = 0, last_region = 0, last_wgs = 0;
	int n_textures = 0, n_tex_mats = 0; long long texel_bytes = 0; int last_textured = 0;
	DevBuf side;
	DevBuf dn_cz[2], dn_nr, dn_stage;
	hipEvent_t dn_ev[2] = { nullptr, nullptr }, gd_ev[2] = { nullptr, nullptr }; bool dn_timed = false, gd_timed = false;
	int last_dn = 0, last_dn_demod = 0, last_guide_spp = 0; float last_dn_sigma[3] = { 0.f, 0.f, 0.f };
	int light_mode = JP_LIGHTS_ALL;
	int n_selectable = 0; double total_weight = 0.0; int last_picked = 0;
	EnvMapHost env_map;
	int env_importance = 0, env_n_selectable = 0; double env_total_weight = 0.0; long long env_table_bytes = 0; int last_mapped = 0;
	int estimator = JP_ESTIMATOR_NEE, last_mis = 0;
	DevBuf mis_side[2];
	VertexNormalsHost vnormals;
	int vn_triangles = 0, vn_smooth = 0, last_smooth = 0; long long vn_table_bytes = 0; double normal_ms = 0.0;
	DevBuf nside;
	NormalMapsHost nmaps;
	int last_nmapped = 0; double normal_map_ms = 0.0;
	TexSamplingHost tsamp;
	int upload_n_textures = 0, last_sampled = 0; double texel_ms = 0.0;
	MipmapsHost mipmaps;
	std::vector<int2> mip_host_tex; std::vector<JpMipLevel> mip_host_lev; double mip_build_ms = 0.0; int last_mip = 0;
	DevBuf cone;
	JpLens lens = {}; bool lens_on = false; int last_lens = 0;
	JpFilm film_state = {}; bool film_on = false; int last_hdr = 0;
	JpToneMap tonemap = {}; bool tonemap_on = false; int last_tonemapped = 0; float last_scale = 0.f;
	DevBuf film_hist, film_stage;
	hipEvent_t fh_ev[2] = { nullptr, nullptr }, tm_ev[2] = { nullptr, nullptr }; bool fh_timed = false, tm_timed = false;
};
// ... 245 lines not shown
```

jet-pbrt_amd/csrc/jp_scene_host.h:

```cpp
#pragma once
namespace
{
struct HV3 { float x, y, z; };
inline HV3 hsub(HV3 a, HV3 b) { HV3 r = { a.x - b.x, a.y - b.y, a.z - b.z }; return r; }
inline HV3 hcross(HV3 a, HV3 v) { HV3 r = { a.y * v.z - a.z * v.y, a.z * v.x - a.x * v.z, a.x * v.y - a.y * v.x }; return r; }
inline float hlen(HV3 a) { return std::sqrt(a.x * a.x + a.y * a.y + a.z * a.z); }
inline HV3 hld(const float* p) { HV3 r = { p[0], p[1], p[2] }; return r; }
inline HV3 hnorm(HV3 a) { const float l = hlen(a); HV3 r = { a.x / l, a.y / l, a.z / l }; return r; }
inline float box_area(const float* b) { float dx = b[3] - b[0], dy = b[4] - b[1], dz = b[5] - b[2]; return dx * dy + dy * dz + dz * dx; }
inline uint32_t pack4(const uint8_t* v) { return (uint32_t)v[0] | ((uint32_t)v[1] << 8) | ((uint32_t)v[2] << 16) | ((uint32_t)v[3] << 24); }
inline uint64_t fnv1a(const void* p, size_t n) { uint64_t h = 1469598103934665603ull; for (size_t i = 0; i < n; i++) { h ^= ((const unsigned char*)p)[i]; h *= 1099511628211ull; } return h; }

struct ItemTree { std::vector<int> left, right; std::vector<float> bounds; int height = 0; };
int item_tree_build(const std::vector<float>& ib, std::vector<int>& idx, int start, int end, ItemTree& t, int depth)
{
	const int node = (int)t.left.size(); t.left.push_back(0); t.right.push_back(0); t.bounds.resize(t.bounds.size() + 6);
	t.height = std::max(t.height, depth);
	float nb[6] = { 1e30f, 1e30f, 1e30f, -1e30f, -1e30f, -1e30f }, cb[6] = { 1e30f, 1e30f, 1e30f, -1e30f, -1e30f, -1e30f };
	for (int i = start; i < end; i++)
	{
		const float* b = &ib[6 * (size_t)idx[i]];
		for (int a = 0; a < 3; a++) { nb[a] = std::min(nb[a], b[a]); nb[3 + a] = std::max(nb[3 + a], b[3 + a]); const float c = 0.5f * (b[a] + b[3 + a]); cb[a] = std::min(cb[a], c); cb[3 + a] = std::max(cb[3 + a], c); }
	}
	std::memcpy(&t.bounds[6 * (size_t)node], nb, sizeof(nb));
// ... 40 lines not shown
	return node;
}

int bvh_height(const JpScene* s, int node, int depth, int limit, bool& bad, std::vector<char>& seen)
{
	if (node < 0 || node >= s->n_bvh_nodes || seen[node] || depth > limit) { bad = true; return 0; }
	seen[node] = 1;
	if (s->bvh_left[node] < 0) return 0;
	int a = bvh_height(s, s->bvh_left[node], depth + 1, limit, bad, seen);
	int b = bvh_height(s, s->bvh_right[node], depth + 1, limit, bad, seen);
	return 1 + std::max(a, b);
}

struct SceneCheck
{
	std::vector<char> seen; int height = 0, n_leaves = 0; bool has_null = false;
	bool device_build = false;
	bool ref_sem = false;
};
int check_scene(const JpScene* s, bool pick, SceneCheck& k)
{
	if (s->n_primitives <= 0) return fail(JP_ERR_INVALID_ARGUMENT, "jp_upload_scene: scene has no primitives");
	if (s->n_triangles < 0 || s->n_rectangles < 0 || s->n_spheres < 0 || s->n_disks < 0 || s->n_materials < 0 || s->n_lights < 0 || s->n_bvh_nodes < 0 || s->n_bvh_prim_indices < 0)
		return fail(JP_ERR_INVALID_ARGUMENT, "jp_upload_scene: negative count");
	if (s->bvh_reference_semantics < 0 || s->bvh_reference_semantics > 2) return fail(JP_ERR_INVALID_ARGUMENT, "jp_upload_scene: bvh_reference_semantics must be 0, 1 or 2");
	if (s->bvh_reference_semantics != 0 && s->n_bvh_nodes == 0) return fail(JP_ERR_INVALID_ARGUMENT, "jp_upload_scene: reference semantics need the caller's tree (n_bvh_nodes == 0)");
	const bool device_build = k.device_build = s->n_bvh_nodes == 0;
	k.ref_sem = !device_build && (s->bvh_reference_semantics == 1 || s->bvh_reference_semantics == 2);
	if (!s->prim_shape_type || !s->prim_shape_index || !s->prim_material || !s->prim_light || (!device_build && (!s->bvh_bounds || !s->bvh_left || !s->bvh_right || !s->bvh_prim_index)))
		return fail(JP_ERR_INVALID_ARGUMENT, "jp_upload_scene: null array");
	if ((s->n_triangles && (!s->tri_p0 || !s->tri_p1 || !s->tri_p2 || !s->tri_n)) || (s->n_rectangles && (!s->rect_p0 || !s->rect_p1 || !s->rect_p2 || !s->rect_p3 || !s->rect_n))
	    || (s->n_spheres && (!s->sph_center || !s->sph_radius)) || (s->n_disks && (!s->disk_center || !s->disk_normal || !s->disk_radius)) || (s->n_materials && (!s->mat_type || !s->mat_params)) || (s->n_lights && (!s->light_type || !s->light_radiance || !s->light_prim)))
		return fail(JP_ERR_INVALID_ARGUMENT, "jp_upload_scene: null array for a non-zero count");
	if (!pick && s->n_lights > 255) return fail(JP_ERR_UNSUPPORTED, "jp_upload_scene: more than 255 lights are not supported by the shadow-entry packing");
	if (pick && s->n_lights > (1 << 24)) return fail(JP_ERR_UNSUPPORTED, "jp_upload_scene: more than 2^24 lights (JP_LIGHTS_POWER_ONE)");
	for (int i = 0; i < s->n_primitives; i++)
	{
		int t = s->prim_shape_type[i], j = s->prim_shape_index[i];
		int lim = t == JP_SHAPE_TRIANGLE ? s->n_triangles : t == JP_SHAPE_RECTANGLE ? s->n_rectangles : t == JP_SHAPE_SPHERE ? s->n_spheres : t == JP_SHAPE_DISK ? s->n_disks : -1;
		if (lim < 0 || j < 0 || j >= lim) return fail(JP_ERR_INVALID_ARGUMENT, "jp_upload_scene: primitive shape reference out of range");
		if (s->prim_material[i] < -1 || s->prim_material[i] >= s->n_materials) return fail(JP_ERR_INVALID_ARGUMENT, "jp_upload_scene: primitive material out of range");
		if (s->prim_light[i] < -1 || s->prim_light[i] >= s->n_lights) return fail(JP_ERR_INVALID_ARGUMENT, "jp_upload_scene: primitive light out of range");
		if (s->prim_light[i] >= 0 && s->light_type[s->prim_light[i]] != JP_LIGHT_AREA) return fail(JP_ERR_INVALID_ARGUMENT, "jp_upload_scene: primitive light is not an area light");
		if (s->prim_material[i] < 0) k.has_null = true;
	}
	for (int i = 0; i < s->n_materials; i++) if (s->mat_type[i] < JP_MAT_MATTE || s->mat_type[i] > JP_MAT_METAL) return fail(JP_ERR_INVALID_ARGUMENT, "jp_upload_scene: unknown material type");
	for (int i = 0; i < s->n_lights; i++)
	{
		if (s->light_type[i] == JP_LIGHT_AREA) { if (s->light_prim[i] < 0 || s->light_prim[i] >= s->n_primitives) return fail(JP_ERR_INVALID_ARGUMENT, "jp_upload_scene: area light primitive out of range"); }
		else if (s->light_type[i] == JP_LIGHT_POINT || s->light_type[i] == JP_LIGHT_DIRECTION) { if (!s->light_vec) return fail(JP_ERR_INVALID_ARGUMENT, "jp_upload_scene: point / direction light without light_vec"); }
		else if (s->light_type[i] != JP_LIGHT_ENVIRONMENT) return fail(JP_ERR_INVALID_ARGUMENT, "jp_upload_scene: unknown light type");
	}
	k.seen.assign(s->n_bvh_nodes, 0); bool bad = false;
	k.height = device_build ? 0 : bvh_height(s, 0, 0, 4 * JP_STACK_DEPTH, bad, k.seen);
	if (bad) return fail(JP_ERR_INVALID_ARGUMENT, "jp_upload_scene: BVH is not a tree rooted at node 0 (cycle, bad child index or excessive depth)");
	if (!device_build && k.height + 1 > JP_STACK_DEPTH) return fail(JP_ERR_INVALID_ARGUMENT, "jp_upload_scene: BVH height exceeds the device traversal stack (32)");
	std::vector<int> primSeen(s->n_primitives, 0);
	for (int n = 0; n < s->n_bvh_nodes; n++)
	{
		if (!k.seen[n] || s->bvh_left[n] >= 0) continue;
		k.n_leaves++;
		int first = -s->bvh_left[n] - 1, cnt = s->bvh_right[n];
		if (cnt < 1 || cnt > 16 || first < 0 || first + cnt > s->n_bvh_prim_indices) return fail(JP_ERR_INVALID_ARGUMENT, "jp_upload_scene: BVH leaf range invalid (1..16 primitives per leaf)");
		for (int j = 0; j < cnt; j++) { int p = s->bvh_prim_index[first + j]; if (p < 0 || p >= s->n_primitives) return fail(JP_ERR_INVALID_ARGUMENT, "jp_upload_scene: BVH primitive index out of range"); primSeen[p]++; }
	}
	if (!device_build) for (int i = 0; i < s->n_primitives; i++) if (primSeen[i] != 1) return fail(JP_ERR_INVALID_ARGUMENT, "jp_upload_scene: every primitive must be in exactly one BVH leaf");
	return JP_OK;
}
int check_leaf_encoding(const JpScene* s)
{
	return (size_t)s->n_primitives >= (1u << 27) ? fail(JP_ERR_UNSUPPORTED, "jp_upload_scene: too many primitives for the leaf reference encoding") : JP_OK;
}

enum { TAB_NODES, TAB_PRIMS, TAB_META, TAB_MATS, TAB_MAT_TYPE, TAB_LIGHTS, TAB_SHADE_TAB, TAB_WIDE, TAB_Q4, TAB_REFBOX, TAB_FLAT, TAB_COUNT };
static_assert(TAB_COUNT == JP_UPLOAD_TABLES, "JpUploadInfo::table lists the host-built tables");
struct TableBytes { const void* data; size_t bytes; bool present; };

struct PlanSizes { int n_nodes, n_prims, n_flat, height, wide_height, q4_height, planes; bool use_wide, use_q4, use_cert, has_null; };

struct HostTables
{
	std::vector<float4> nodes, prims, refbox, flat, mats, lights, shade_tab; std::vector<int4> meta; std::vector<uint32_t> wide, q4; std::vector<int> mat_type;
	std::vector<int> devPrimOf;
	std::vector<float> light_area;
	bool device_build = false, use_wide = false, use_q4 = false, use_cert = false, has_null = false;
	int n_nodes = 0, n_wide = 0, n_q4 = 0;
	int height = 0, wide_height = 0, q4_height = 0, eye_leaves = 0, n_env = 0, planes = 0;
	float cert_pad = 0.f, cert_pad_eye = 0.f, env_sum[3] = { 0.f, 0.f, 0.f };
	PlanSizes sizes() const { PlanSizes z = { n_nodes, (int)meta.size(), (int)(flat.size() / 2), height, wide_height, q4_height, planes, use_wide, use_q4, use_cert, has_null }; return z; }
	void tables(TableBytes r[TAB_COUNT]) const
	{
		auto some = [](const auto& v, bool on) { TableBytes b = { v.data(), on ? v.size() * sizeof(v[0]) : 0, on }; return b; };
		r[TAB_NODES] = some(nodes, !device_build); r[TAB_PRIMS] = some(prims, !device_build); r[TAB_META] = some(meta, !device_build);
		r[TAB_MATS] = some(mats, true); r[TAB_MAT_TYPE] = some(mat_type, true); r[TAB_LIGHTS] = some(lights, true); r[TAB_SHADE_TAB] = some(shade_tab, true);
		r[TAB_WIDE] = some(wide, !wide.empty()); r[TAB_Q4] = some(q4, !q4.empty()); r[TAB_REFBOX] = some(refbox, !refbox.empty()); r[TAB_FLAT] = some(flat, !flat.empty());
	}
};

struct RecordEmitter
{
	const JpScene* s; float extra_pad;
	std::vector<float4>& prims; std::vector<int4>& meta; std::vector<int>& devPrimOf;
	RecordEmitter(const JpScene* scene, const JpOptions& op, HostTables& t) : s(scene), extra_pad(std::max(0.f, op.box_pad)), prims(t.prims), meta(t.meta), devPrimOf(t.devPrimOf) { devPrimOf.assign(s->n_primitives, -1); }
	void padded_box(const float* src, float* b) const
	{
		for (int a = 0; a < 3; a++)
		{
			float lo = src[a], hi = src[3 + a];
			float m = std::max(std::fabs(lo), std::fabs(hi)); float e = m * 1e-6f + 1e-6f + extra_pad;
			b[a] = lo - e; b[3 + a] = hi + e;
		}
	}
	void node_box(int n, float* b) const { padded_box(s->bvh_bounds + 6 * (size_t)n, b); }
	int emit_prim(int p)
	{
		const int dev = (int)meta.size(); devPrimOf[p] = dev;
		int t = s->prim_shape_type[p], i = s->prim_shape_index[p];
		float4 g[4] = { make_float4(0, 0, 0, 0), make_float4(0, 0, 0, 0), make_float4(0, 0, 0, 0), make_float4(0, 0, 0, 0) };
		if (t == JP_SHAPE_TRIANGLE)
		{
			g[0] = make_float4(s->tri_p0[3 * i], s->tri_p0[3 * i + 1], s->tri_p0[3 * i + 2], 0); g[1] = make_float4(s->tri_p1[3 * i], s->tri_p1[3 * i + 1], s->tri_p1[3 * i + 2], 0);
			g[2] = make_float4(s->tri_p2[3 * i], s->tri_p2[3 * i + 1], s->tri_p2[3 * i + 2], 0); g[3] = make_float4(s->tri_n[3 * i], s->tri_n[3 * i + 1], s->tri_n[3 * i + 2], 0);
		}
		else if (t == JP_SHAPE_RECTANGLE)
		{
			g[0] = make_float4(s->rect_p0[3 * i], s->rect_p0[3 * i + 1], s->rect_p0[3 * i + 2], s->rect_p3[3 * i]);
			g[1] = make_float4(s->rect_p1[3 * i], s->rect_p1[3 * i + 1], s->rect_p1[3 * i + 2], s->rect_p3[3 * i + 1]);
			g[2] = make_float4(s->rect_p2[3 * i], s->rect_p2[3 * i + 1], s->rect_p2[3 * i + 2], s->rect_p3[3 * i + 2]);
			g[3] = make_float4(s->rect_n[3 * i], s->rect_n[3 * i + 1], s->rect_n[3 * i + 2], 0);
		}
		else if (t == JP_SHAPE_DISK)
		{
			g[0] = make_float4(s->disk_center[3 * i], s->disk_center[3 * i + 1], s->disk_center[3 * i + 2], s->disk_radius[i]);
			g[1] = make_float4(s->disk_normal[3 * i], s->disk_normal[3 * i + 1], s->disk_normal[3 * i + 2], 0);
		}
		else g[0] = make_float4(s->sph_center[3 * i], s->sph_center[3 * i + 1], s->sph_center[3 * i + 2], s->sph_radius[i]);
		int tb = t; std::memcpy(&g[3].w, &tb, 4);
		for (int j = 0; j < 4; j++) prims.push_back(g[j]);
		int4 m; m.x = p; m.y = s->prim_material[p]; m.z = s->prim_light[p]; m.w = t; meta.push_back(m);
		return dev;
	}
	int emit_leaf(int n)
	{
		int first = -s->bvh_left[n] - 1, cnt = s->bvh_right[n];
		int dfirst = devPrimOf[s->bvh_prim_index[first]];
		if (dfirst < 0) { dfirst = (int)meta.size(); for (int k = 0; k < cnt; k++) emit_prim(s->bvh_prim_index[first + k]); }
		return -(((dfirst << 4) | (cnt - 1)) + 1);
	}
};

inline void quantise_scale(const float* lo, const float* hi, int eb[3], float sc3[3])
{
	for (int a = 0; a < 3; a++)
	{
		int e = (int)std::ceil(std::log2(std::max((hi[a] - lo[a]) / 255.f, 1e-30f)));
		e = std::max(-120, std::min(120, e));
		eb[a] = e + 127; sc3[a] = std::ldexp(1.0f, e);
	}
}
struct QuantAxis { uint8_t q0, q1; bool lo_ok, hi_ok; };
inline QuantAxis quantise_box_axis(float blo, float bhi, float lo, float sc)
{
	int q0 = (int)std::floor((blo - lo) / sc), q1 = (int)std::ceil((bhi - lo) / sc);
	q0 = std::max(0, std::min(255, q0)); q1 = std::max(0, std::min(255, q1));
	while (q0 > 0 && std::fmaf((float)q0, sc, lo) > blo) q0--;
	while (q1 < 255 && std::fmaf((float)q1, sc, lo) < bhi) q1++;
// ... 239 lines not shown
	{
		const float* b = &lv.box[6 * (size_t)i];
		for (int k = 0; k < lv.cnt[i]; k++) { const size_t p = (size_t)lv.first[i] + k; t.refbox[2 * p] = make_float4(b[0], b[1], b[2], 0.f); t.refbox[2 * p + 1] = make_float4(b[3], b[4], b[5], 0.f); }
		diag += std::sqrt((double)(b[3] - b[0]) * (b[3] - b[0]) + (double)(b[4] - b[1]) * (b[4] - b[1]) + (double)(b[5] - b[2]) * (b[5] - b[2]));
	}
	const float K = op.cert_slack == 0.f ? 16384.f : std::max(0.f, op.cert_slack);
	t.cert_pad = (float)(K * 1.1920929e-7 / std::max(1e-20, diag / ni));
	const float Ke = op.cert_slack_eye == 0.f ? std::min(K, 1024.f) : std::max(0.f, op.cert_slack_eye);
	t.cert_pad_eye = (float)(Ke * 1.1920929e-7 / std::max(1e-20, diag / ni));
	return true;
}

void build_flat(const RecordEmitter& em, const SceneCheck& k, std::vector<float4>& flat)
{
	const JpScene* s = em.s;
	if (s->n_primitives > 64 || k.n_leaves > 32) return;
	for (int n = 0; n < s->n_bvh_nodes; n++)
	{
		if (!k.seen[n] || s->bvh_left[n] >= 0) continue;
		float bb[6]; em.node_box(n, bb);
		int first = -s->bvh_left[n] - 1, cnt = s->bvh_right[n];
		unsigned long long bits = 0;
		for (int j = 0; j < cnt; j++) bits |= 1ull << em.devPrimOf[s->bvh_prim_index[first + j]];
		const uint32_t lo = (uint32_t)bits, hi = (uint32_t)(bits >> 32); float flo, fhi; std::memcpy(&flo, &lo, 4); std::memcpy(&fhi, &hi, 4);
		flat.push_back(make_float4(bb[0], bb[1], bb[2], flo)); flat.push_back(make_float4(bb[3], bb[4], bb[5], fhi));
	}
}

void build_material_light_tables(const JpScene* s, bool pick, HostTables& t)
{
	t.mats.assign(4 * (size_t)std::max(1, s->n_materials), make_float4(0, 0, 0, 0)); t.mat_type.assign(std::max(1, s->n_materials), 0);
	for (int i = 0; i < s->n_materials; i++) { std::memcpy(&t.mats[4 * i], s->mat_params + (size_t)i * JP_MAT_PARAM_STRIDE, 16 * sizeof(float)); t.mat_type[i] = s->mat_type[i]; }
	t.lights.assign(2 * (size_t)std::max(1, s->n_lights), make_float4(0, 0, 0, 0)); t.planes = t.n_env = 0; t.env_sum[0] = t.env_sum[1] = t.env_sum[2] = 0.f;
	t.light_area.assign(pick ? (size_t)s->n_lights : 0, 0.f);
	for (int i = 0; i < s->n_lights; i++)
	{
		int ty = s->light_type[i]; float tf; std::memcpy(&tf, &ty, 4);
		const float* rad = s->light_radiance + 3 * i;
		t.lights[2 * i] = make_float4(rad[0], rad[1], rad[2], tf);
		bool black = rad[0] == 0.f && rad[1] == 0.f && rad[2] == 0.f;
		if (!black) t.planes++;
		float inv_area = 0.f; int dp = -1;
		if (ty == JP_LIGHT_AREA)
		{
			int p = s->light_prim[i]; dp = t.devPrimOf[p];
			int st = s->prim_shape_type[p], k = s->prim_shape_index[p]; float area;
			if (st == JP_SHAPE_TRIANGLE) area = 0.5f * hlen(hcross(hsub(hld(s->tri_p1 + 3 * k), hld(s->tri_p0 + 3 * k)), hsub(hld(s->tri_p2 + 3 * k), hld(s->tri_p0 + 3 * k))));
			else if (st == JP_SHAPE_RECTANGLE) area = hlen(hcross(hsub(hld(s->rect_p0 + 3 * k), hld(s->rect_p1 + 3 * k)), hsub(hld(s->rect_p2 + 3 * k), hld(s->rect_p1 + 3 * k))));
			else if (st == JP_SHAPE_DISK) { const float kPi = (float)3.14159265358979323846; area = kPi * s->disk_radius[k] * s->disk_radius[k]; }
			else { const float kPi = (float)3.14159265358979323846; float r2 = s->sph_radius[k] * s->sph_radius[k]; area = 4 * kPi * r2; }
			inv_area = 1 / area;
			if (pick) t.light_area[i] = area;
		}
		else if (ty == JP_LIGHT_ENVIRONMENT) { t.n_env++; t.env_sum[0] += rad[0]; t.env_sum[1] += rad[1]; t.env_sum[2] += rad[2]; }
		float df; std::memcpy(&df, &dp, 4);
		t.lights[2 * i + 1] = make_float4(df, inv_area, 0, 0);
		if (ty == JP_LIGHT_POINT || ty == JP_LIGHT_DIRECTION) t.lights[2 * i + 1] = make_float4(s->light_vec[3 * i], s->light_vec[3 * i + 1], s->light_vec[3 * i + 2], 0);
	}
}

void build_shade_tab(const JpScene* s, bool pick, HostTables& t)
{
	std::vector<float4>& tabv = t.shade_tab; tabv.clear();
	if (!pick) tabv.insert(tabv.end(), t.lights.begin(), t.lights.begin() + 2 * (size_t)s->n_lights);
	tabv.insert(tabv.end(), t.mats.begin(), t.mats.begin() + 4 * (size_t)s->n_materials);
	const size_t at = tabv.size(); tabv.resize(at + ((size_t)s->n_materials + 3) / 4, make_float4(0, 0, 0, 0));
	if (s->n_materials > 0) std::memcpy(&tabv[at], t.mat_type.data(), (size_t)s->n_materials * sizeof(int));
	if (t.device_build) return;
	tabv.insert(tabv.end(), t.prims.begin(), t.prims.end());
	const size_t am = tabv.size(); tabv.resize(am + t.meta.size());
	std::memcpy(&tabv[am], t.meta.data(), t.meta.size() * sizeof(int4));
	for (size_t pi = 0; pi < t.meta.size(); pi++)
	{
		const float4 g3 = t.prims[4 * pi + 3], g1 = t.prims[4 * pi + 1];
		int type; std::memcpy(&type, &g3.w, 4);
		const HV3 nn = type == JP_SHAPE_DISK ? HV3{ g1.x, g1.y, g1.z } : HV3{ g3.x, g3.y, g3.z };
		const HV3 n = hnorm(nn);
		const HV3 tmp = std::fabs(n.x) > 0.99f ? HV3{ 0, 1, 0 } : HV3{ 1, 0, 0 };
		const HV3 tg = hnorm(hcross(n, tmp)), sv = hnorm(hcross(tg, n));
		tabv.push_back(make_float4(n.x, n.y, n.z, 0)); tabv.push_back(make_float4(sv.x, sv.y, sv.z, 0)); tabv.push_back(make_float4(tg.x, tg.y, tg.z, 0));
	}
}

int build_host_tables(const JpScene* s, const JpOptions& op, bool pick, const SceneCheck& k, HostTables& t)
{
	if (const int st = check_leaf_encoding(s); st != JP_OK) return st;
	RecordEmitter em(s, op, t);
	t.height = k.height; t.has_null = k.has_null;
	const bool inner_root = s->bvh_left[0] >= 0;
	if (k.ref_sem)
	{
		LeafItems leaves;
		build_reference_nodes(em, t.nodes, leaves);
		const bool want_cert = s->bvh_reference_semantics == 2 && op.certified >= 0 && s->n_primitives > 1024 && leaves.first.size() >= 64;
		t.use_cert = want_cert && build_certified(em, op, leaves, t);
	}
	else
	{
		t.use_wide = k.n_leaves > 32 && inner_root;
		if (((size_t)s->n_bvh_nodes + (size_t)s->n_primitives) * 80 + (size_t)(k.height + 2) * JP_BLOCK * sizeof(int) <= 40 * 1024) t.use_wide = false;
		if (op.traversal > 0) { const int m = op.traversal - 1; if (m == 3 && inner_root) t.use_wide = true; else if (m >= 0 && m <= 2) t.use_wide = false; }
		if (t.use_wide && (!build_wide8(em, t.wide, t.wide_height) || (int)t.meta.size() != s->n_primitives))
		{
			t.use_wide = false; t.wide.clear(); t.prims.clear(); t.meta.clear(); std::fill(t.devPrimOf.begin(), t.devPrimOf.end(), -1);
		}
		build_binary(em, t.nodes);
		t.use_q4 = s->n_primitives > 1024 && inner_root && opt_flag(op.q4, true);
		if (t.use_q4 && (!build_q4(em, t.q4, t.q4_height) || (int)t.meta.size() != s->n_primitives)) { t.use_q4 = false; t.q4.clear(); }
		build_flat(em, k, t.flat);
	}
	t.n_nodes = (int)(t.nodes.size() / 4); t.n_wide = (int)(t.wide.size() / 20); t.n_q4 = (int)(t.q4.size() / 16);
	build_material_light_tables(s, pick, t);
	build_shade_tab(s, pick, t);
	return JP_OK;
}

int build_light_table(int n, const double* w, float* q, int32_t* alias, float* pmf, double* W_out, int* n_sel_out)
{
	double W = 0.0; int nsel = 0;
	for (int i = 0; i < n; i++)
	{
		if (!(w[i] >= 0.0) || !std::isfinite(w[i])) return fail(JP_ERR_INVALID_ARGUMENT, "jp_build_light_table: a weight is negative or not finite");
		W += w[i]; if (w[i] > 0.0) nsel++;
	}
	if (W_out) *W_out = std::isfinite(W) ? W : 0.0;
	if (n_sel_out) *n_sel_out = nsel;
	if (!std::isfinite(W)) return fail(JP_ERR_INVALID_ARGUMENT, "jp_build_light_table: the weights' sum is not finite");
	if (!(W > 0.0))
	{
		for (int i = 0; i < n; i++) { if (q) q[i] = 0.f; if (alias) alias[i] = i; if (pmf) pmf[i] = 0.f; }
		return JP_OK;
	}
	std::vector<double> p((size_t)n); std::vector<int> small, large, al((size_t)n); std::vector<float> th((size_t)n);
	small.reserve((size_t)n); large.reserve((size_t)n);
	for (int i = 0; i < n; i++) { p[i] = w[i] * (double)n / W; al[i] = i; th[i] = 1.f; }
	for (int i = n - 1; i >= 0; i--) if (w[i] > 0.0 && p[i] < 1.0) small.push_back(i);
	for (int i = n - 1; i >= 0; i--) if (w[i] == 0.0) small.push_back(i);
	for (int i = n - 1; i >= 0; i--) if (p[i] >= 1.0) large.push_back(i);
	while (!small.empty() && !large.empty())
	{
		const int s = small.back(); small.pop_back();
		const int l = large.back();
		th[s] = (float)p[s]; al[s] = l;
		p[l] = (p[l] + p[s]) - 1.0;
		if (p[l] < 1.0) { large.pop_back(); small.push_back(l); }
	}
	for (int s : small) if (w[s] == 0.0) return fail(JP_ERR_INVALID_ARGUMENT, "jp_build_light_table: weights too extreme for the table");
	for (int i = 0; i < n; i++)
	{
		if (q) q[i] = th[i];
		if (alias) alias[i] = al[i];
		if (pmf) pmf[i] = (float)(w[i] / W);
	}
	return JP_OK;
}

int check_environment_map(const char* who, const JpEnvMap* m)
{
	const std::string w(who);
	if (m->struct_bytes < (int32_t)sizeof(JpEnvMap)) return fail(JP_ERR_INVALID_ARGUMENT, w + ": set JpEnvMap.struct_bytes to sizeof(JpEnvMap)");
	if (m->width < 1 || m->width > 4096 || m->height < 1 || m->height > 4096) return fail(JP_ERR_INVALID_ARGUMENT, w + ": map size out of range (1 .. 4096 per side)");
	if (m->up_axis != JP_ENV_UP_Z && m->up_axis != JP_ENV_UP_Y) return fail(JP_ERR_INVALID_ARGUMENT, w + ": unknown up_axis");
	if (m->importance != 0 && m->importance != -1) return fail(JP_ERR_INVALID_ARGUMENT, w + ": importance must be 0 or -1");
	if (!m->rgb) return fail(JP_ERR_INVALID_ARGUMENT, w + ": null rgb");
	const size_t n = 3 * (size_t)m->width * m->height;
	for (size_t i = 0; i < n; i++) if (!(m->rgb[i] >= 0.f) || !std::isfinite(m->rgb[i])) return fail(JP_ERR_INVALID_ARGUMENT, w + ": a texel value is negative or not finite");
	return JP_OK;
}
struct EnvTables
{
	std::vector<double> weight; std::vector<float> q; std::vector<int32_t> alias; std::vector<float4> texel; std::vector<float2> row_cos;
	double total = 0.0, mean_sum = 0.0; int n_selectable = 0;
};
int build_environment_table(const JpEnvMap* m, const float* tint, EnvTables& e)
{
	if (const int st = check_environment_map("jp_build_environment_table", m); st != JP_OK) return st;
	for (int k = 0; k < 3; k++) if (!(tint[k] >= 0.f) || !std::isfinite(tint[k])) return fail(JP_ERR_INVALID_ARGUMENT, "jp_build_environment_table: the tint is negative or not finite");
	const double kPi = 3.14159265358979323846;
	const int W = m->width, H = m->height; const size_t n = (size_t)W * H;
	e.weight.resize(n); e.q.resize(n); e.alias.resize(n); e.texel.resize(n); e.row_cos.resize((size_t)H);
	std::vector<double> omega((size_t)H);
	double lum = 0.0;
	for (int r = 0; r < H; r++)
	{
		const double ct = std::cos(kPi * (double)r / (double)H), cb = std::cos(kPi * (double)(r + 1) / (double)H);
		omega[r] = (2.0 * kPi / (double)W) * (ct - cb);
		e.row_cos[r] = make_float2((float)ct, (float)cb);
		for (int c = 0; c < W; c++)
		{
			const size_t t = (size_t)r * W + c;
			const float R = tint[0] * m->rgb[3 * t], G = tint[1] * m->rgb[3 * t + 1], B = tint[2] * m->rgb[3 * t + 2];
			if (!std::isfinite(R) || !std::isfinite(G) || !std::isfinite(B)) return fail(JP_ERR_INVALID_ARGUMENT, "jp_build_environment_table: tint x texel is not finite");
			const double s = (((double)R + (double)G) + (double)B) * omega[r];
			lum += s;
			e.weight[t] = m->importance == -1 ? omega[r] : s;
			e.texel[t] = make_float4(R, G, B, 0.f);
		}
	}
	if (const int st = build_light_table((int)n, e.weight.data(), e.q.data(), e.alias.data(), nullptr, &e.total, &e.n_selectable); st != JP_OK) return st;
	if (e.total > 0.0) for (size_t t = 0; t < n; t++) e.texel[t].w = (float)((e.weight[t] / e.total) / omega[t / (size_t)W]);
	e.mean_sum = lum / (4.0 * kPi);
	return JP_OK;
}

ScenePlan plan_scene(const JpScene* s, const JpOptions& op, bool pick, bool device_build, const PlanSizes& z)
{
	ScenePlan p;
	const bool ref_sem = !device_build && s->bvh_reference_semantics != 0;
	p.cert = z.use_cert;
	p.use_q4 = z.use_q4; p.q4_shadow = z.use_q4 && opt_flag(op.q4_shadow, true);
	p.stack_depth = std::max(2, z.height + 2);
	p.stack_depth_q4 = (z.use_q4 || z.use_cert) ? 3 * z.q4_height + 2 : 0;
	const size_t scene_bytes = ((size_t)z.n_nodes + (size_t)z.n_prims) * 5 * sizeof(float4);
	const size_t prim_bytes = (size_t)z.n_prims * 5 * sizeof(float4);
	const size_t stack_bytes = (size_t)p.stack_depth * JP_BLOCK * sizeof(int);
	p.scene_in_lds = !device_build && scene_bytes + stack_bytes <= 40 * 1024;
	p.trav_mode = z.use_wide ? 3 : ((z.n_flat > 0 && prim_bytes <= 40 * 1024) ? 2 : (p.scene_in_lds ? 1 : 0));
	if (!z.use_wide && op.traversal > 0) { const int m = op.traversal - 1; if (m == 0 || (m == 1 && p.scene_in_lds)) p.trav_mode = m; }
	if (z.use_wide) p.scene_in_lds = false;
	if (ref_sem) p.trav_mode = 5;
	p.lds_bytes = p.trav_mode == 2 ? prim_bytes : (p.trav_mode == 1 ? stack_bytes + scene_bytes : stack_bytes);
	p.lds_bytes_shadow = p.trav_mode == 3 ? (size_t)2 * (z.wide_height + 2) * JP_BLOCK * sizeof(int) : p.lds_bytes;
	{
		const int planes = pick ? std::min(z.planes, 1) : z.planes;
		size_t tab = ((pick ? (size_t)0 : (size_t)2 * s->n_lights) + (size_t)4 * s->n_materials) * sizeof(float4) + (size_t)s->n_materials * sizeof(int) + 16;
		p.tables_in_lds = tab <= 16 * 1024;
		const size_t shade_static = (size_t)JP_SHADE_TILE * 3 + (size_t)JP_SHADE_CLASSES * (JP_SHADE_TILE / JP_BLOCK) * (JP_BLOCK / 64) * 4 + 128;
		const size_t prim_part = (size_t)z.n_prims * (4 * sizeof(float4) + sizeof(int4) + 3 * sizeof(float4));
		p.shade_prims_in_lds = p.tables_in_lds && p.scene_in_lds && tab + prim_part <= 24 * 1024;
		p.shade_lds_bytes = p.tables_in_lds ? tab + (p.shade_prims_in_lds ? prim_part : 0) : 0;
		const size_t stage_bytes = 16 + (size_t)std::max(1, planes) * 2 * JP_BLOCK * sizeof(float4);
		p.stage_nee = p.tables_in_lds && std::max(1, planes) <= 4 && shade_static + p.shade_lds_bytes + stage_bytes <= 64 * 1024;
		if (p.stage_nee) p.shade_lds_bytes += stage_bytes;
		p.n_planes = std::max(1, planes);
	}
	bool kinds[8] = { false, false, false, false, false, false, false, false }; int nk = 0;
	for (int i = 0; i < s->n_primitives; i++) { const int m = s->prim_material[i]; const int k = m < 0 ? 7 : s->mat_type[m]; if (!kinds[k]) { kinds[k] = true; nk++; } }
	p.stack_lds_words = op.stack_lds_words >= 2 ? (op.stack_lds_words & ~1) : 12;
	p.persist = ((p.trav_mode == 0 || p.trav_mode == 3 || p.trav_mode == 5) && s->n_primitives > 1024) ? 16 : 0;
	if (op.persist != 0) p.persist = op.persist < 0 ? 0 : op.persist;
	p.vote = opt_flag(op.vote, p.trav_mode != 5 || p.cert);
	p.class_mask = 1; for (int k = 0; k < 5; k++) if (kinds[k]) p.class_mask |= 2 << k;
	p.shade_sort = opt_flag(op.shade_sort, nk > 1);
	p.shape_mask = 0; p.light_mask = 0; p.light_shape_mask = 0;
	for (int i = 0; i < s->n_primitives; i++) p.shape_mask |= 1 << (s->prim_shape_type[i] & 3);
	for (int i = 0; i < s->n_lights; i++)
	{
		const float* rad = s->light_radiance + 3 * i;
		if (rad[0] == 0.f && rad[1] == 0.f && rad[2] == 0.f) continue;
		p.light_mask |= 1 << (s->light_type[i] & 3);
		if (s->light_type[i] == JP_LIGHT_AREA) p.light_shape_mask |= 1 << (s->prim_shape_type[s->light_prim[i]] & 3);
	}
	p.has_null_material = z.has_null;
	return p;
}
}
```

jet-pbrt_amd/csrc/jp_upload.h:

```cpp
#pragma once
namespace
{
int device_build_tables(JpContext* c, const JpScene* s, bool pick, const SceneCheck& k, HostTables& t, SceneTables& T, float& build_ms)
{
	const JpOptions& op = c->opt;
	if (const int st = check_leaf_encoding(s); st != JP_OK) return st;
	RecordEmitter em(s, op, t);
	t.device_build = true; t.has_null = k.has_null;
	for (int p = 0; p < s->n_primitives; p++) em.emit_prim(p);
	DevBuf p0, m0; float4* d_p0; int4* d_m0;
	hipError_t e = reserve(p0, d_p0, t.prims.size() * sizeof(float4)); if (e == hipSuccess) e = reserve(m0, d_m0, t.meta.size() * sizeof(int4));
	if (e == hipSuccess) e = hipMemcpyAsync(d_p0, t.prims.data(), t.prims.size() * sizeof(float4), hipMemcpyHostToDevice, c->stream);
	if (e == hipSuccess) e = hipMemcpyAsync(d_m0, t.meta.data(), t.meta.size() * sizeof(int4), hipMemcpyHostToDevice, c->stream);
	LbvhResult lr; std::vector<int> sorted;
	bool ploc = op.device_tree != 2;
	int maxLeaf = ploc ? 2 : 3;
	if (op.bvh_max_leaf >= 1 && op.bvh_max_leaf <= 16) maxLeaf = op.bvh_max_leaf;
	if (e == hipSuccess && ploc) { e = ploc_build(c->stream, d_p0, d_m0, s->n_primitives, maxLeaf, op.ploc_radius, op.ploc_max_rounds, lr, sorted); if (e == hipErrorNotReady) { e = hipSuccess; ploc = false; } }
	if (e == hipSuccess && !ploc) e = lbvh_build(c->stream, d_p0, d_m0, s->n_primitives, maxLeaf, lr, sorted);
	p0.reset(); m0.reset();
	if (e != hipSuccess) return fail(JP_ERR_DEVICE, std::string("jp_upload_scene: device BVH build failed: ") + hipGetErrorString(e));
	if (lr.height + 2 > 60) return fail(JP_ERR_UNSUPPORTED, "jp_upload_scene: device-built BVH is deeper than the 58-entry traversal stack; hand over a host-built hierarchy for this scene");
	T.nodes = std::move(lr.nodes); T.prims = std::move(lr.prims); T.meta = std::move(lr.meta);
	for (int i = 0; i < s->n_primitives; i++) t.devPrimOf[sorted[i]] = i;
	t.height = lr.height; build_ms = lr.build_ms; t.n_nodes = lr.n_nodes;
	const bool want_wide = opt_flag(op.device_wide, s->n_primitives > 64);
	if (want_wide)
	{
		WideResult wr;
		e = lbvh_build_wide(c->stream, T.nodes.get<float4>(), s->n_primitives, wr);
		if (e != hipSuccess) return fail(JP_ERR_DEVICE, std::string("jp_upload_scene: device wide-tree build failed: ") + hipGetErrorString(e));
		if (wr.wide) { T.wide = std::move(wr.wide); t.n_wide = wr.n_wide; t.wide_height = wr.height; t.use_wide = true; build_ms += wr.build_ms; }
	}
	const bool want_q4 = s->n_primitives > 1024 && opt_flag(op.q4, true);
	if (want_q4)
	{
		WideResult qr;
		e = lbvh_build_q4(c->stream, T.nodes.get<float4>(), s->n_primitives, qr);
		if (e != hipSuccess) return fail(JP_ERR_DEVICE, std::string("jp_upload_scene: device 4-wide tree build failed: ") + hipGetErrorString(e));
		if (qr.wide) { T.q4 = std::move(qr.wide); t.n_q4 = qr.n_wide; build_ms += qr.build_ms; t.use_q4 = true; t.q4_height = qr.height; }
	}
	build_material_light_tables(s, pick, t);
	build_shade_tab(s, pick, t);
	return JP_OK;
}

void bind_scene_view(SceneView& v, const SceneTables& T, const HostTables& t, const JpScene* s)
{
	v.nodes = T.nodes.get<float4>(); v.n_nodes = t.n_nodes;
	v.prims = T.prims.get<float4>(); v.meta = T.meta.get<int4>(); v.n_prims = (int)t.meta.size();
	v.mats = T.mats.get<float4>(); v.mat_type = T.mat_type.get<int>(); v.n_mats = s->n_materials;
	v.lights = T.lights.get<float4>(); v.n_lights = s->n_lights; v.shade_tab = T.shade_tab.get<float4>();
	v.env_sum = make_float3(t.env_sum[0], t.env_sum[1], t.env_sum[2]); v.n_env = t.n_env;
	v.world_radius = s->world_radius; v.cam = s->camera;
	v.flat = T.flat.get<float4>(); v.n_flat = (int)(t.flat.size() / 2);
	v.wide = T.wide.get<uint4>(); v.n_wide = t.n_wide;
	v.q4 = T.q4.get<uint4>(); v.n_q4 = t.n_q4;
	v.refbox = T.refbox.get<float4>(); v.cert_pad = t.cert_pad; v.cert_pad_eye = t.cert_pad_eye;
}
}

extern "C" int jp_upload_scene(JpContext* c, const JpScene* s)
{
	if (!c || !s) return fail(JP_ERR_INVALID_ARGUMENT, "jp_upload_scene: null argument");
	const bool pick = c->light_mode == JP_LIGHTS_POWER_ONE;
	SceneCheck k;
	if (const int st = check_scene(s, pick, k); st != JP_OK) return st;
	const int n_textures = c->upload_n_textures; c->upload_n_textures = 0;
	if (const int st = check_sampling_counts(c, n_textures); st != JP_OK) return st;
	if (const int st = check_mipmap_counts(c, n_textures); st != JP_OK) return st;
	HIP_TRY(hipSetDevice(c->device));
	HIP_TRY(hipStreamSynchronize(c->stream));
	free_scene(c);

	HostTables t; SceneTables T; float build_ms = 0.f;
	if (const int st = k.device_build ? device_build_tables(c, s, pick, k, t, T, build_ms) : build_host_tables(s, c->opt, pick, k, t); st != JP_OK) return st;
	static DevBuf SceneTables::* const kDst[TAB_COUNT] = { &SceneTables::nodes, &SceneTables::prims, &SceneTables::meta, &SceneTables::mats, &SceneTables::mat_type, &SceneTables::lights,
	                                                        &SceneTables::shade_tab, &SceneTables::wide, &SceneTables::q4, &SceneTables::refbox, &SceneTables::flat };
	TableBytes tb[TAB_COUNT]; t.tables(tb);
	for (int i = 0; i < TAB_COUNT; i++) if (tb[i].present) HIP_TRY(upload(T.*kDst[i], tb[i].data, tb[i].bytes));
	ScenePlan p = plan_scene(s, c->opt, pick, k.device_build, t.sizes());
	bind_scene_view(p.sv, T, t, s);
	if (c->env_map.W > 0) { if (const int st = upload_environment_map(c, T, p, s, pick); st != JP_OK) return st; c->env_importance = c->env_map.importance; }
	if (pick) if (const int st = upload_light_table(c, T, p, s, t.light_area); st != JP_OK) return st;
	if (c->vnormals.set) if (const int st = upload_vertex_normals(c, T, p, s); st != JP_OK) return st;
	if (c->nmaps.set) if (const int st = upload_normal_maps(c, T, p, s); st != JP_OK) return st;
	if (const int st = upload_map_sampling(c, T, p); st != JP_OK) return st;

	c->tab = std::move(T); c->plan = p; c->plan.have_scene = true;
	c->build_on_device = k.device_build; c->build_ms = build_ms; c->bvh_height = t.height; c->bvh_nodes = k.ref_sem ? s->n_bvh_nodes : t.n_nodes;
	c->cert_eye_leaves = t.eye_leaves; c->cert_fell_back = false;
	for (int i = 0; i < TAB_COUNT; i++) c->tab_bytes[i] = tb[i].present ? tb[i].bytes : 0;
	if (k.device_build)
	{
		c->tab_bytes[TAB_NODES] = (size_t)t.n_nodes * 4 * sizeof(float4); c->tab_bytes[TAB_PRIMS] = (size_t)s->n_primitives * 4 * sizeof(float4); c->tab_bytes[TAB_META] = (size_t)s->n_primitives * sizeof(int4);
		c->tab_bytes[TAB_WIDE] = (size_t)t.n_wide * 20 * sizeof(uint32_t); c->tab_bytes[TAB_Q4] = (size_t)t.n_q4 * 16 * sizeof(uint32_t);
	}
	c->wide_height = t.wide_height; c->q4_height = t.q4_height;
	return JP_OK;
}

namespace
{
int host_upload_tables(const std::string& who, const JpOptions* o, int32_t light_mode, const JpScene* s, JpOptions& op, SceneCheck& k, HostTables& t)
{
	if (light_mode != JP_LIGHTS_ALL && light_mode != JP_LIGHTS_POWER_ONE) return fail(JP_ERR_INVALID_ARGUMENT, who + ": unknown light sampling mode");
	std::memset(&op, 0, sizeof(op)); op.struct_bytes = (int32_t)sizeof(JpOptions);
	if (o) if (const int st = read_options(who.c_str(), o, op); st != JP_OK) return st;
	const bool pick = light_mode == JP_LIGHTS_POWER_ONE;
	if (const int st = check_scene(s, pick, k); st != JP_OK) return st;
	if (k.device_build) return fail(JP_ERR_UNSUPPORTED, who + ": a scene without a hierarchy (n_bvh_nodes == 0) gets its trees from the device builders");
	return build_host_tables(s, op, pick, k, t);
}
}

extern "C" int jp_describe_upload(const JpOptions* o, int32_t light_mode, const JpScene* s, JpUploadInfo* out)
{
	if (!s || !out) return fail(JP_ERR_INVALID_ARGUMENT, "jp_describe_upload: null argument");
	if (out->struct_bytes < (int32_t)sizeof(int32_t)) return fail(JP_ERR_INVALID_ARGUMENT, "jp_describe_upload: set JpUploadInfo.struct_bytes to sizeof(JpUploadInfo)");
	JpOptions op; SceneCheck k; HostTables t;
	if (const int st = host_upload_tables("jp_describe_upload", o, light_mode, s, op, k, t); st != JP_OK) return st;
	const bool pick = light_mode == JP_LIGHTS_POWER_ONE;
	const ScenePlan p = plan_scene(s, op, pick, false, t.sizes());
	JpUploadInfo i; std::memset(&i, 0, sizeof(i));
	i.trav_mode = p.trav_mode; i.stack_depth = p.stack_depth; i.stack_depth_q4 = p.stack_depth_q4;
	i.lds_bytes = (int64_t)p.lds_bytes; i.lds_bytes_shadow = (int64_t)p.lds_bytes_shadow; i.shade_lds_bytes = (int64_t)p.shade_lds_bytes;
	i.scene_in_lds = p.scene_in_lds; i.tables_in_lds = p.tables_in_lds; i.shade_prims_in_lds = p.shade_prims_in_lds; i.stage_nee = p.stage_nee; i.n_planes = p.n_planes;
	i.persist = p.persist; i.vote = p.vote; i.shade_sort = p.shade_sort; i.use_q4 = p.use_q4; i.q4_shadow = p.q4_shadow; i.cert = p.cert;
	i.class_mask = p.class_mask; i.shape_mask = p.shape_mask; i.light_mask = p.light_mask; i.light_shape_mask = p.light_shape_mask;
	i.has_null_material = p.has_null_material; i.stack_lds_words = p.stack_lds_words;
	i.n_nodes = t.n_nodes; i.n_prims = (int32_t)t.meta.size(); i.n_flat = (int32_t)(t.flat.size() / 2); i.n_wide = t.n_wide; i.n_q4 = t.n_q4;
	i.bvh_nodes = k.ref_sem ? s->n_bvh_nodes : t.n_nodes; i.bvh_height = t.height; i.wide_height = t.wide_height; i.q4_height = t.q4_height;
	i.cert_eye_leaves = p.cert ? t.eye_leaves : 0; i.n_env = t.n_env;
	i.cert_pad = t.cert_pad; i.cert_pad_eye = t.cert_pad_eye; std::memcpy(i.env_sum, t.env_sum, sizeof(i.env_sum));
	TableBytes tb[TAB_COUNT]; t.tables(tb);
	for (int j = 0; j < TAB_COUNT; j++) if (tb[j].present) { i.table[j].bytes = (int64_t)tb[j].bytes; i.table[j].fnv1a = fnv1a(tb[j].data, tb[j].bytes); }
	const size_t n = std::min((size_t)out->struct_bytes, sizeof(i));
	i.struct_bytes = (int32_t)n;
	std::memcpy(out, &i, n);
	return JP_OK;
}

extern "C" int jp_copy_upload_table(const JpOptions* o, int32_t light_mode, const JpScene* s, int32_t which, void* out, int64_t capacity_bytes, int64_t* bytes)
{
	if (!s || !bytes) return fail(JP_ERR_INVALID_ARGUMENT, "jp_copy_upload_table: null argument");
	if (which < 0 || which >= TAB_COUNT) return fail(JP_ERR_INVALID_ARGUMENT, "jp_copy_upload_table: no such table");
	JpOptions op; SceneCheck k; HostTables t;
	if (const int st = host_upload_tables("jp_copy_upload_table", o, light_mode, s, op, k, t); st != JP_OK) return st;
	TableBytes tb[TAB_COUNT]; t.tables(tb);
	*bytes = tb[which].present ? (int64_t)tb[which].bytes : 0;
	if (!out) return JP_OK;
	if (capacity_bytes < *bytes) return fail(JP_ERR_INVALID_ARGUMENT, "jp_copy_upload_table: capacity_bytes smaller than the table");
	if (*bytes > 0) std::memcpy(out, tb[which].data, (size_t)*bytes);
	return JP_OK;
}

extern "C" int jp_read_scene_table(JpContext* c, int32_t which, void* out, int64_t capacity_bytes, int64_t* bytes)
{
	if (!c || !bytes) return fail(JP_ERR_INVALID_ARGUMENT, "jp_read_scene_table: null argument");
	if (!c->plan.have_scene) return fail(JP_ERR_NO_SCENE, "jp_read_scene_table: no scene uploaded");
	const DevBuf* src = which == TAB_NODES ? &c->tab.nodes : which == TAB_PRIMS ? &c->tab.prims : which == TAB_META ? &c->tab.meta : which == TAB_WIDE ? &c->tab.wide
	                  : which == TAB_Q4 ? &c->tab.q4 : which == TAB_FLAT ? &c->tab.flat : nullptr;
	if (!src) return fail(JP_ERR_INVALID_ARGUMENT, "jp_read_scene_table: not a hierarchy table (nodes, prims, meta, wide, q4, flat)");
	*bytes = (int64_t)c->tab_bytes[which];
	if ((size_t)*bytes > src->bytes()) return fail(JP_ERR_DEVICE, "jp_read_scene_table: the table is larger than its device buffer");
	if (!out) return JP_OK;
	if (capacity_bytes < *bytes) return fail(JP_ERR_INVALID_ARGUMENT, "jp_read_scene_table: capacity_bytes smaller than the table");
	HIP_TRY(hipSetDevice(c->device));
	HIP_TRY(hipStreamSynchronize(c->stream));
	if (*bytes > 0) HIP_TRY(hipMemcpy(out, src->get<void>(), (size_t)*bytes, hipMemcpyDeviceToHost));
	return JP_OK;
}
extern "C" int jp_get_tree_info(JpContext* c, JpTreeInfo* out)
{
	if (!c || !out) return fail(JP_ERR_INVALID_ARGUMENT, "jp_get_tree_info: null argument");
	if (out->struct_bytes < (int32_t)sizeof(int32_t)) return fail(JP_ERR_INVALID_ARGUMENT, "jp_get_tree_info: set JpTreeInfo.struct_bytes to sizeof(JpTreeInfo)");
	if (!c->plan.have_scene) return fail(JP_ERR_NO_SCENE, "jp_get_tree_info: no scene uploaded");
	const SceneView& v = c->plan.sv;
	JpTreeInfo i; std::memset(&i, 0, sizeof(i));
	i.n_prims = v.n_prims; i.n_nodes = v.n_nodes; i.bvh_height = c->bvh_height;
	i.n_wide = v.n_wide; i.wide_height = c->wide_height; i.n_q4 = v.n_q4; i.q4_height = c->q4_height; i.n_flat = v.n_flat;
	const size_t n = std::min((size_t)out->struct_bytes, sizeof(i));
	i.struct_bytes = (int32_t)n;
	std::memcpy(out, &i, n);
	return JP_OK;
}


namespace
{
int check_textures(const JpScene* s, const JpTextures* t, long long& pool, int& ntm)
{
	pool = 0; ntm = 0;
	if (t->struct_bytes < (int32_t)sizeof(JpTextures)) return fail(JP_ERR_INVALID_ARGUMENT, "jp_upload_scene_textured: JpTextures.struct_bytes smaller than this library's JpTextures");
	if (t->n_textures < 0 || t->n_textures > (1 << 28)) return fail(JP_ERR_INVALID_ARGUMENT, "jp_upload_scene_textured: n_textures out of range");
	const int nt = t->n_textures;
	if (nt == 0) return JP_OK;
	if (!t->tex_type || !t->tex_color) return fail(JP_ERR_INVALID_ARGUMENT, "jp_upload_scene_textured: null tex_type / tex_color");
	if (t->n_materials != s->n_materials) return fail(JP_ERR_INVALID_ARGUMENT, "jp_upload_scene_textured: n_materials differs from the scene's");
	if (t->n_triangles != s->n_triangles) return fail(JP_ERR_INVALID_ARGUMENT, "jp_upload_scene_textured: n_triangles differs from the scene's");
	if (t->n_materials > 0 && (!t->mat_texture || !s->mat_type)) return fail(JP_ERR_INVALID_ARGUMENT, "jp_upload_scene_textured: null mat_texture");
	for (int i = 0; i < nt; i++)
	{
		const int ty = t->tex_type[i];
		if (ty < JP_TEXTURE_SOLID || ty > JP_TEXTURE_IMAGE) return fail(JP_ERR_INVALID_ARGUMENT, "jp_upload_scene_textured: unknown texture type");
		if (ty == JP_TEXTURE_IMAGE)
		{
			if (!t->tex_width || !t->tex_height || !t->tex_offset || !t->texels) return fail(JP_ERR_INVALID_ARGUMENT, "jp_upload_scene_textured: image texture without tex_width / tex_height / tex_offset / texels");
			const long long w = t->tex_width[i], h = t->tex_height[i], off = t->tex_offset[i];
			if (w < 1 || w > 16384 || h < 1 || h > 16384) return fail(JP_ERR_INVALID_ARGUMENT, "jp_upload_scene_textured: image size out of range (1 .. 16384 per side)");
			if (off < 0 || t->n_texel_bytes < 0 || off > t->n_texel_bytes - 3 * w * h) return fail(JP_ERR_INVALID_ARGUMENT, "jp_upload_scene_textured: image texels beyond n_texel_bytes");
			pool += w * h;
		}
		else
		{
			const int nc = ty == JP_TEXTURE_CHECKER ? 6 : 3;
			for (int k = 0; k < nc; k++) if (!std::isfinite(t->tex_color[6 * (size_t)i + k])) return fail(JP_ERR_INVALID_ARGUMENT, "jp_upload_scene_textured: colour not finite");
		}
	}
	if (pool > 0x7fffffffll) return fail(JP_ERR_INVALID_ARGUMENT, "jp_upload_scene_textured: more than 2^31 texels in all");
	for (int m = 0; m < t->n_materials; m++)
	{
		const int k = t->mat_texture[m];
		if (k < -1 || k >= nt) return fail(JP_ERR_INVALID_ARGUMENT, "jp_upload_scene_textured: mat_texture out of range");
		if (k < 0) continue;
		const int mt = s->mat_type[m];
		if (mt != JP_MAT_MATTE && mt != JP_MAT_MIRROR && mt != JP_MAT_PLASTIC) return fail(JP_ERR_INVALID_ARGUMENT, "jp_upload_scene_textured: a texture on a glass or metal material (its [0..2] is eta, not a colour)");
		ntm++;
	}
	if (s->n_primitives > 0 && (!s->prim_shape_type || !s->prim_shape_index)) return fail(JP_ERR_INVALID_ARGUMENT, "jp_upload_scene_textured: null array");
	return JP_OK;
}
struct TexTables { std::vector<int4> desc; std::vector<float4> col; std::vector<unsigned int> texels; std::vector<int> mat_tex; std::vector<float2> prim_uv; };
void build_texture_tables(const JpScene* s, const JpTextures* t, long long pool, TexTables& x)
{
	const int nt = t->n_textures;
	std::vector<int4>& desc = x.desc; std::vector<float4>& col = x.col; std::vector<unsigned int>& texels = x.texels;
	desc.resize(nt); col.resize(2 * (size_t)nt); texels.resize((size_t)pool);
	size_t at = 0;
	for (int i = 0; i < nt; i++)
	{
		const float* cc = t->tex_color + 6 * (size_t)i;
		desc[i] = make_int4(t->tex_type[i], 0, 0, 0);
		col[2 * i] = make_float4(0, 0, 0, 0); col[2 * i + 1] = make_float4(0, 0, 0, 0);
		if (t->tex_type[i] == JP_TEXTURE_IMAGE)
		{
			const int w = t->tex_width[i], h = t->tex_height[i];
// ... 55 lines not shown
```

Baseline: 3547.

## Precompute per-primitive shading class table and prefetch hit prims for sort

Builds a byte-per-primitive table of shading class (material type + 1, or 0 for null) on the host. It uploads the table in front of the shade table and optionally stages it in LDS. The shade kernel's sort passes now read one byte per hit instead of chasing meta then mat_type, and the hit primitive indices are loaded into registers up front, before the table staging loop. This cuts dependent global loads in the classification step, at the cost of more registers, a bit more LDS, and new API plumbing for reading the table.

```diff
diff --git a/include/jetpbrt_amd.h b/include/jetpbrt_amd.h
--- a/include/jetpbrt_amd.h
+++ b/include/jetpbrt_amd.h
@@ -402,7 +402,7 @@
 } JpUploadInfo;
 int  jp_describe_upload(const JpOptions* options_or_null, int32_t light_mode, const JpScene* scene, JpUploadInfo* out);
 
-enum { JP_TABLE_NODES = 0, JP_TABLE_PRIMS = 1, JP_TABLE_META = 2, JP_TABLE_WIDE = 7, JP_TABLE_Q4 = 8, JP_TABLE_FLAT = 10 };
+enum { JP_TABLE_NODES = 0, JP_TABLE_PRIMS = 1, JP_TABLE_META = 2, JP_TABLE_WIDE = 7, JP_TABLE_Q4 = 8, JP_TABLE_FLAT = 10, JP_TABLE_CLASS = 16 };
 typedef struct JpTreeInfo {
     int32_t struct_bytes;
     int32_t n_prims, n_nodes, bvh_height;
diff --git a/jet-pbrt_amd/__init__.py b/jet-pbrt_amd/__init__.py
--- a/jet-pbrt_amd/__init__.py
+++ b/jet-pbrt_amd/__init__.py
@@ -610,7 +610,12 @@
                 ("n_q4", C.c_int32), ("q4_height", C.c_int32), ("n_flat", C.c_int32)]
 
 
+JP_TABLE_CLASS = 16
+
+
 def _table_index(which):
+    if which == "class_of_prim":
+        return JP_TABLE_CLASS
     return UPLOAD_TABLES.index(which) if isinstance(which, str) else int(which)
 
 
diff --git a/jet-pbrt_amd/csrc/jp_kernels.hip b/jet-pbrt_amd/csrc/jp_kernels.hip
--- a/jet-pbrt_amd/csrc/jp_kernels.hip
+++ b/jet-pbrt_amd/csrc/jp_kernels.hip
@@ -237,6 +237,32 @@
 {
 	if constexpr (kSmooth) return sm.guard && dot(w, Ng) * dot(wo, Ng) <= 0.f; else return false;
 }
+constexpr int kShadeGroups = JP_SHADE_TILE / JP_BLOCK / 8;
+static_assert(JP_SHADE_TILE % (8 * JP_BLOCK) == 0, "k_shade: a region is whole groups of eight passes");
+__device__ __forceinline__ void region_prims(const float2* hit, unsigned int count, unsigned int npass, int (&pi)[8 * kShadeGroups])
+{
+	const char* base = (const char*)hit + 4;
+	#pragma unroll
+	for (int g = 0; g < kShadeGroups; g++)
+		if (8u * g < npass)
+		{
+			#pragma unroll
+			for (int u = 0; u < 8; u++)
+			{
+				const unsigned int j = (8u * g + u) * JP_BLOCK + threadIdx.x;
+				pi[8 * g + u] = *(const int*)(base + 8u * (j < count ? j : count - 1u));
+			}
+		}
+}
+__device__ __forceinline__ void group_keys(const unsigned char* cls, const int (&pi)[8 * kShadeGroups], int g, unsigned int count, unsigned int (&key)[8])
+{
+	unsigned int c[8];
+	#pragma unroll
+	for (int u = 0; u < 8; u++) c[u] = cls[pi[8 * g + u] < 0 ? 0 : pi[8 * g + u]];
+	#pragma unroll
+	for (int u = 0; u < 8; u++) key[u] = (8u * g + u) * JP_BLOCK + threadIdx.x < count ? (pi[8 * g + u] >= 0 ? c[u] : 0u) : (unsigned int)JP_SHADE_CLASSES;
+}
+
 template <bool kTab, bool kPrims, bool kStage, bool kSort, bool kTex, bool kPick, bool kEnv, bool kMis, typename F = FeatAll, bool kOne = false, bool kSmooth = false>
 __device__ __forceinline__ void shade_body(SceneView sc, Queues q, RenderConst rc, int cur, DevCounters* cnt, const TexView& tv, const PickView& pv, const EnvView& ev, const MisView& mv, const NormView& nv = NormView())
 {
@@ -255,8 +281,10 @@
 	__shared__ unsigned int s_ctr[3];
 	const unsigned int lane = threadIdx.x & 63u;
 	const int n_tab_l = kPick ? 0 : 2 * sc.n_lights;
-	const int n_tab = n_tab_l + 4 * sc.n_mats + (sc.n_mats + 3) / 4, n_tab_all = n_tab + (kPrims ? 8 * sc.n_prims : 0);
-	float4* s_lights = s_dyn;
+	const int n_cls = kSort ? (sc.n_prims + 15) / 16 : 0, n_cls_lds = kPrims ? n_cls : 0;
+	const int n_tab = n_cls_lds + n_tab_l + 4 * sc.n_mats + (sc.n_mats + 3) / 4, n_tab_all = n_tab + (kPrims ? 8 * sc.n_prims : 0);
+	const unsigned char* class_of_prim = kPrims ? (const unsigned char*)s_dyn : (const unsigned char*)(sc.shade_tab - n_cls);
+	float4* s_lights = s_dyn + n_cls_lds;
 	float4* s_mats = s_lights + n_tab_l;
 	int* s_mtype = (int*)(s_mats + 4 * sc.n_mats);
 	float4* s_prims = s_dyn + n_tab;
@@ -268,12 +296,15 @@
 #ifdef JP_SHADE_TIMING
 	unsigned long long t_acc[10] = { 0, 0, 0, 0, 0, 0, 0, 0, 0, 0 }, t_last = __builtin_amdgcn_s_memtime();
 #endif
+	int hit_prim[8 * kShadeGroups];
+	if constexpr (kSort) region_prims(q.hit + b * q.R, n, (n + JP_BLOCK - 1) / JP_BLOCK, hit_prim);
 	if (kTab)
 	{
+		const float4* tab = sc.shade_tab - n_cls_lds;
 		for (int i = threadIdx.x; i < n_tab_all; i += 2 * JP_BLOCK)
 		{
 			const bool two = i + JP_BLOCK < n_tab_all;
-			const float4 a = sc.shade_tab[i], c2 = two ? sc.shade_tab[i + JP_BLOCK] : a;
+			const float4 a = tab[i], c2 = two ? tab[i + JP_BLOCK] : a;
 			s_dyn[i] = a; if (two) s_dyn[i + JP_BLOCK] = c2;
 		}
 	}
@@ -292,24 +323,18 @@
 	{
 		const unsigned int tid = threadIdx.x, npass = (count + JP_BLOCK - 1) / JP_BLOCK;
 		const unsigned long long ltm = (1ull << lane) - 1ull;
-		#pragma unroll 1
-		for (unsigned int r0 = 0; r0 < npass; r0 += 8)
-		{
-			int pi[8];
-			#pragma unroll
-			for (int u = 0; u < 8; u++)
-			{
-				const unsigned int j = (r0 + u) * JP_BLOCK + tid;
-				pi[u] = j < count ? __float_as_int(q.hit[rbase + t0 + j].y) : -2;
-			}
-			int mt[8]; unsigned long long ma[8], mb[8];
+		#pragma unroll
+		for (int g = 0; g < kShadeGroups; g++)
+		{
+			const unsigned int r0 = 8u * g;
+			if (r0 >= npass) break;
+			unsigned int key[8]; unsigned long long ma[8], mb[8];
+			group_keys(class_of_prim, hit_prim, g, count, key);
 			unsigned int na = 0, nb = 0;
 			#pragma unroll
 			for (int u = 0; u < 8; u++)
 			{
-				mt[u] = -1;
-				if (pi[u] >= 0) { const int m = meta_t[pi[u]].y; if (m >= 0) mt[u] = mat_type[m]; }
-				ma[u] = __ballot(mt[u] == JP_MAT_MATTE); mb[u] = __ballot(mt[u] == JP_MAT_METAL);
+				ma[u] = __ballot(key[u] == 1u + JP_MAT_MATTE); mb[u] = __ballot(key[u] == 1u + JP_MAT_METAL);
 				na += (unsigned int)__popcll(ma[u]); nb += (unsigned int)__popcll(mb[u]);
 			}
 			if (na | nb)
@@ -320,8 +345,8 @@
 				for (int u = 0; u < 8; u++)
 				{
 					const unsigned short j = (unsigned short)((r0 + u) * JP_BLOCK + tid);
-					if (mt[u] == JP_MAT_MATTE) s_idx[a + (unsigned int)__popcll(ma[u] & ltm)] = j;
-					if (mt[u] == JP_MAT_METAL) s_idx[count - 1u - (m + (unsigned int)__popcll(mb[u] & ltm))] = j;
+					if (key[u] == 1u + JP_MAT_MATTE) s_idx[a + (unsigned int)__popcll(ma[u] & ltm)] = j;
+					if (key[u] == 1u + JP_MAT_METAL) s_idx[count - 1u - (m + (unsigned int)__popcll(mb[u] & ltm))] = j;
 					a += (unsigned int)__popcll(ma[u]); m += (unsigned int)__popcll(mb[u]);
 				}
 			}
@@ -334,27 +359,19 @@
 		const unsigned int tid = threadIdx.x;
 		const unsigned int plane = tid & 63u, wave = tid >> 6, npass = (count + JP_BLOCK - 1) / JP_BLOCK;
 		const unsigned long long ltm = (1ull << plane) - 1ull;
-		#pragma unroll 1
-		for (unsigned int r0 = 0; r0 < npass; r0 += 8)
-		{
-			int pi[8];
+		#pragma unroll
+		for (int g = 0; g < kShadeGroups; g++)
+		{
+			const unsigned int r0 = 8u * g;
+			if (r0 >= npass) break;
+			unsigned int keys[8];
+			group_keys(class_of_prim, hit_prim, g, count, keys);
 			#pragma unroll
 			for (int u = 0; u < 8; u++)
 			{
-				const unsigned int j = (r0 + u) * JP_BLOCK + tid;
-				pi[u] = j < count ? __float_as_int(q.hit[rbase + t0 + j].y) : -2;
-			}
-			#pragma unroll
-			for (int u = 0; u < 8; u++)
-			{
 				const unsigned int r = r0 + u;
 				if (r >= npass) break;
-				unsigned int key = JP_SHADE_CLASSES;
-				if (pi[u] != -2)
-				{
-					int m = -1; if (pi[u] >= 0) m = meta_t[pi[u]].y;
-					key = m >= 0 ? 1u + (unsigned int)mat_type[m] : 0u;
-				}
+				const unsigned int key = keys[u];
 				s_key[r * JP_BLOCK + tid] = (unsigned char)key;
 				unsigned int mine = 0;
 				#pragma unroll
diff --git a/jet-pbrt_amd/csrc/jp_normal_map.h b/jet-pbrt_amd/csrc/jp_normal_map.h
--- a/jet-pbrt_amd/csrc/jp_normal_map.h
+++ b/jet-pbrt_amd/csrc/jp_normal_map.h
@@ -223,7 +223,7 @@
 	if (!plan.smooth)
 	{
 		plan.nv = NormView(); plan.smooth = true;
-		plan.tables_in_lds = false; plan.shade_prims_in_lds = false; plan.stage_nee = false; plan.shade_lds_bytes = 0;
+		plan.tables_in_lds = false; plan.shade_prims_in_lds = false; plan.stage_nee = false; plan.shade_lds_bytes = 0; plan.shade_class_bytes = 0;
 	}
 	return JP_OK;
 }
diff --git a/jet-pbrt_amd/csrc/jp_normals.h b/jet-pbrt_amd/csrc/jp_normals.h
--- a/jet-pbrt_amd/csrc/jp_normals.h
+++ b/jet-pbrt_amd/csrc/jp_normals.h
@@ -141,7 +141,7 @@
 	HIP_TRY(upload(T.prim_vn, rec.data(), rec.size() * sizeof(float4)));
 	plan.nv = NormView(); plan.nv.prim_vn = T.prim_vn.get<float4>();
 	plan.smooth = true;
-	plan.tables_in_lds = false; plan.shade_prims_in_lds = false; plan.stage_nee = false; plan.shade_lds_bytes = 0;
+	plan.tables_in_lds = false; plan.shade_prims_in_lds = false; plan.stage_nee = false; plan.shade_lds_bytes = 0; plan.shade_class_bytes = 0;
 	c->vn_table_bytes = (long long)(rec.size() * sizeof(float4));
 	return JP_OK;
 }
diff --git a/jet-pbrt_amd/csrc/jp_render.h b/jet-pbrt_amd/csrc/jp_render.h
--- a/jet-pbrt_amd/csrc/jp_render.h
+++ b/jet-pbrt_amd/csrc/jp_render.h
@@ -333,7 +333,7 @@
 					Stamper t(c, CLS_SHADE);
 					if (tex) launch_texel(c, p, grid, cur, tv, mv_cone);
 					if (smooth) launch_normal(c, p, grid, cur, nv);
-					shade(c->stream, grid, p.shade_lds_bytes, p.sv, c->q, rc, cur, d_cnt);
+					shade(c->stream, grid, p.shade_lds_bytes + p.shade_class_bytes, p.sv, c->q, rc, cur, d_cnt);
 				}
 				HIP_TRY(hipGetLastError());
 				if (it < rp->max_depth || p.has_null_material)
diff --git a/jet-pbrt_amd/csrc/jp_runtime.h b/jet-pbrt_amd/csrc/jp_runtime.h
--- a/jet-pbrt_amd/csrc/jp_runtime.h
+++ b/jet-pbrt_amd/csrc/jp_runtime.h
@@ -54,7 +54,7 @@
 	bool use_q4 = false, q4_shadow = false;
 	bool vote = false; int persist = 0;
 	int n_planes = 1; bool has_null_material = false;
-	bool tables_in_lds = false, stage_nee = false; size_t shade_lds_bytes = 0;
+	bool tables_in_lds = false, stage_nee = false; size_t shade_lds_bytes = 0, shade_class_bytes = 0;
 	int class_mask = 0x3f; bool shade_sort = false;
 	int shape_mask = 0xf, light_mask = 0xf, light_shape_mask = 0xf;
 	int stack_lds_words = 12;
diff --git a/jet-pbrt_amd/csrc/jp_scene_host.h b/jet-pbrt_amd/csrc/jp_scene_host.h
--- a/jet-pbrt_amd/csrc/jp_scene_host.h
+++ b/jet-pbrt_amd/csrc/jp_scene_host.h
@@ -146,6 +146,7 @@
 {
 	std::vector<float4> nodes, prims, refbox, flat, mats, lights, shade_tab; std::vector<int4> meta; std::vector<uint32_t> wide, q4; std::vector<int> mat_type;
 	std::vector<int> devPrimOf;
+	std::vector<unsigned char> class_tab;
 	std::vector<float> light_area;
 	bool device_build = false, use_wide = false, use_q4 = false, use_cert = false, has_null = false;
 	int n_nodes = 0, n_wide = 0, n_q4 = 0;
@@ -551,6 +552,17 @@
 	}
 }
 
+void build_class_tab(HostTables& t)
+{
+	const size_t n = t.meta.size();
+	t.class_tab.assign((n + 15) / 16 * 16, 0);
+	for (size_t p = 0; p < n; p++)
+	{
+		const int m = t.meta[p].y;
+		t.class_tab[t.device_build ? (size_t)t.devPrimOf[p] : p] = (unsigned char)(m >= 0 ? 1 + t.mat_type[m] : 0);
+	}
+}
+
 int build_host_tables(const JpScene* s, const JpOptions& op, bool pick, const SceneCheck& k, HostTables& t)
 {
 	if (const int st = check_leaf_encoding(s); st != JP_OK) return st;
@@ -581,6 +593,7 @@
 	t.n_nodes = (int)(t.nodes.size() / 4); t.n_wide = (int)(t.wide.size() / 20); t.n_q4 = (int)(t.q4.size() / 16);
 	build_material_light_tables(s, pick, t);
 	build_shade_tab(s, pick, t);
+	build_class_tab(t);
 	return JP_OK;
 }
 
@@ -696,10 +709,12 @@
 		p.tables_in_lds = tab <= 16 * 1024;
 		const size_t shade_static = (size_t)JP_SHADE_TILE * 3 + (size_t)JP_SHADE_CLASSES * (JP_SHADE_TILE / JP_BLOCK) * (JP_BLOCK / 64) * 4 + 128;
 		const size_t prim_part = (size_t)z.n_prims * (4 * sizeof(float4) + sizeof(int4) + 3 * sizeof(float4));
-		p.shade_prims_in_lds = p.tables_in_lds && p.scene_in_lds && tab + prim_part <= 24 * 1024;
+		const size_t class_part = ((size_t)z.n_prims + 15) / 16 * 16;
+		p.shade_prims_in_lds = p.tables_in_lds && p.scene_in_lds && tab + prim_part + class_part <= 24 * 1024;
 		p.shade_lds_bytes = p.tables_in_lds ? tab + (p.shade_prims_in_lds ? prim_part : 0) : 0;
+		p.shade_class_bytes = p.shade_prims_in_lds ? class_part : 0;
 		const size_t stage_bytes = 16 + (size_t)std::max(1, planes) * 2 * JP_BLOCK * sizeof(float4);
-		p.stage_nee = p.tables_in_lds && std::max(1, planes) <= 4 && shade_static + p.shade_lds_bytes + stage_bytes <= 64 * 1024;
+		p.stage_nee = p.tables_in_lds && std::max(1, planes) <= 4 && shade_static + p.shade_lds_bytes + p.shade_class_bytes + stage_bytes <= 64 * 1024;
 		if (p.stage_nee) p.shade_lds_bytes += stage_bytes;
 		p.n_planes = std::max(1, planes);
 	}
diff --git a/jet-pbrt_amd/csrc/jp_upload.h b/jet-pbrt_amd/csrc/jp_upload.h
--- a/jet-pbrt_amd/csrc/jp_upload.h
+++ b/jet-pbrt_amd/csrc/jp_upload.h
@@ -42,7 +42,16 @@
 	}
 	build_material_light_tables(s, pick, t);
 	build_shade_tab(s, pick, t);
-	return JP_OK;
+	build_class_tab(t);
+	return JP_OK;
+}
+
+hipError_t upload_shade_tables(DevBuf& b, const HostTables& t)
+{
+	std::vector<unsigned char> all(t.class_tab);
+	const unsigned char* tab = (const unsigned char*)t.shade_tab.data();
+	all.insert(all.end(), tab, tab + t.shade_tab.size() * sizeof(float4));
+	return upload(b, all.data(), all.size());
 }
 
 void bind_scene_view(SceneView& v, const SceneTables& T, const HostTables& t, const JpScene* s)
@@ -50,7 +59,7 @@
 	v.nodes = T.nodes.get<float4>(); v.n_nodes = t.n_nodes;
 	v.prims = T.prims.get<float4>(); v.meta = T.meta.get<int4>(); v.n_prims = (int)t.meta.size();
 	v.mats = T.mats.get<float4>(); v.mat_type = T.mat_type.get<int>(); v.n_mats = s->n_materials;
-	v.lights = T.lights.get<float4>(); v.n_lights = s->n_lights; v.shade_tab = T.shade_tab.get<float4>();
+	v.lights = T.lights.get<float4>(); v.n_lights = s->n_lights; v.shade_tab = T.shade_tab.get<float4>() + t.class_tab.size() / sizeof(float4);
 	v.env_sum = make_float3(t.env_sum[0], t.env_sum[1], t.env_sum[2]); v.n_env = t.n_env;
 	v.world_radius = s->world_radius; v.cam = s->camera;
 	v.flat = T.flat.get<float4>(); v.n_flat = (int)(t.flat.size() / 2);
@@ -78,7 +87,7 @@
 	static DevBuf SceneTables::* const kDst[TAB_COUNT] = { &SceneTables::nodes, &SceneTables::prims, &SceneTables::meta, &SceneTables::mats, &SceneTables::mat_type, &SceneTables::lights,
 	                                                        &SceneTables::shade_tab, &SceneTables::wide, &SceneTables::q4, &SceneTables::refbox, &SceneTables::flat };
 	TableBytes tb[TAB_COUNT]; t.tables(tb);
-	for (int i = 0; i < TAB_COUNT; i++) if (tb[i].present) HIP_TRY(upload(T.*kDst[i], tb[i].data, tb[i].bytes));
+	for (int i = 0; i < TAB_COUNT; i++) if (tb[i].present) HIP_TRY(i == TAB_SHADE_TAB ? upload_shade_tables(T.shade_tab, t) : upload(T.*kDst[i], tb[i].data, tb[i].bytes));
 	ScenePlan p = plan_scene(s, c->opt, pick, k.device_build, t.sizes());
 	bind_scene_view(p.sv, T, t, s);
 	if (c->env_map.W > 0) { if (const int st = upload_environment_map(c, T, p, s, pick); st != JP_OK) return st; c->env_importance = c->env_map.importance; }
@@ -144,14 +153,16 @@
 extern "C" int jp_copy_upload_table(const JpOptions* o, int32_t light_mode, const JpScene* s, int32_t which, void* out, int64_t capacity_bytes, int64_t* bytes)
 {
 	if (!s || !bytes) return fail(JP_ERR_INVALID_ARGUMENT, "jp_copy_upload_table: null argument");
-	if (which < 0 || which >= TAB_COUNT) return fail(JP_ERR_INVALID_ARGUMENT, "jp_copy_upload_table: no such table");
+	const bool cls = which == JP_TABLE_CLASS;
+	if (!cls && (which < 0 || which >= TAB_COUNT)) return fail(JP_ERR_INVALID_ARGUMENT, "jp_copy_upload_table: no such table");
 	JpOptions op; SceneCheck k; HostTables t;
 	if (const int st = host_upload_tables("jp_copy_upload_table", o, light_mode, s, op, k, t); st != JP_OK) return st;
 	TableBytes tb[TAB_COUNT]; t.tables(tb);
-	*bytes = tb[which].present ? (int64_t)tb[which].bytes : 0;
+	const TableBytes src = cls ? TableBytes{ t.class_tab.data(), t.meta.size(), true } : tb[which];
+	*bytes = src.present ? (int64_t)src.bytes : 0;
 	if (!out) return JP_OK;
 	if (capacity_bytes < *bytes) return fail(JP_ERR_INVALID_ARGUMENT, "jp_copy_upload_table: capacity_bytes smaller than the table");
-	if (*bytes > 0) std::memcpy(out, tb[which].data, (size_t)*bytes);
+	if (*bytes > 0) std::memcpy(out, src.data, (size_t)*bytes);
 	return JP_OK;
 }
 
@@ -160,9 +171,9 @@
 	if (!c || !bytes) return fail(JP_ERR_INVALID_ARGUMENT, "jp_read_scene_table: null argument");
 	if (!c->plan.have_scene) return fail(JP_ERR_NO_SCENE, "jp_read_scene_table: no scene uploaded");
 	const DevBuf* src = which == TAB_NODES ? &c->tab.nodes : which == TAB_PRIMS ? &c->tab.prims : which == TAB_META ? &c->tab.meta : which == TAB_WIDE ? &c->tab.wide
-	                  : which == TAB_Q4 ? &c->tab.q4 : which == TAB_FLAT ? &c->tab.flat : nullptr;
+	                  : which == TAB_Q4 ? &c->tab.q4 : which == TAB_FLAT ? &c->tab.flat : which == JP_TABLE_CLASS ? &c->tab.shade_tab : nullptr;
 	if (!src) return fail(JP_ERR_INVALID_ARGUMENT, "jp_read_scene_table: not a hierarchy table (nodes, prims, meta, wide, q4, flat)");
-	*bytes = (int64_t)c->tab_bytes[which];
+	*bytes = which == JP_TABLE_CLASS ? (int64_t)c->plan.sv.n_prims : (int64_t)c->tab_bytes[which];
 	if ((size_t)*bytes > src->bytes()) return fail(JP_ERR_DEVICE, "jp_read_scene_table: the table is larger than its device buffer");
 	if (!out) return JP_OK;
 	if (capacity_bytes < *bytes) return fail(JP_ERR_INVALID_ARGUMENT, "jp_read_scene_table: capacity_bytes smaller than the table");
```

After: 3555, median of 4. No clear change (+0.2%).
